# facebookresearch/visual_inertial_bundle_adjustment

Hardware: AMD Instinct MI355X
Metric: LM iterations/sec on 10k-pose/300k-landmark VI-BA (higher is better)
Workload: dtype f64; 1 GPU; config C: 5941186 obs, 300000 landmarks, 10000 rigs, reduced order 150483; rigs=10000, landmarks=300000, observations=5941186, parallelism=single GPU

## Files before the change

### visual_inertial_bundle_adjustment_amd/csrc/api.hip

```cpp
#include "host.hpp"

namespace viba {
ProfSlot g_prof;
}

namespace viba_host {

enum { KF_VISUAL_LIN = 0, KF_LANDMARK, KF_SCHUR, KF_POTRF, KF_GEMM, KF_FWD, KF_BWD, KF_BACKSUB, KF_VISUAL_COST,
       KF_SMALL, KF_TRSM, KF_SYMV, KF_COUNT };

inline void profBegin(vb_handle h, int fam) {
  if (h->profFamily != fam) return;
  if (h->profUsed + 2 > h->profEv.size()) {
    for (int i = 0; i < 256; i++) {
      hipEvent_t e;
      (void)hipEventCreate(&e);
      h->profEv.push_back(e);
    }
  }
  g_prof.start = h->profEv[h->profUsed], g_prof.stop = h->profEv[h->profUsed + 1], g_prof.consumed = false;
}
inline void profEnd(vb_handle h, int fam) {
  if (h->profFamily != fam) return;
  if (g_prof.consumed) h->profUsed += 2;
// ... 370 lines not shown
                          h->st));
    Dev g = d;
    g.tiles = h->tilesGS;
    const Sched& S = h->sch[0];
    launch_potrf(g, S.potrfTileD, S.potrfColD, (int)S.lvP[S.nLevels], h->dinv, h->st);
    launch_trsm(g, S.trsmDiagD, S.trsmTargetD, S.trsmColD, (int)S.lvT[S.nLevels], h->dinv, h->st);
    launch_diag_inverse(g, S.potrfColD, S.lvP[S.nLevels], h->linv, h->st);
  } else if (h->solverType == VB_SOLVER_PCG_LOWER_PREC) {
    return lpInit(h);
  }
  return 0;
}

int precondApply(vb_handle h, const double* r, double* z) {
  Dev& d = h->d;
  const size_t bytes = (size_t)d.nT * TS * sizeof(double);
  if (h->solverType == VB_SOLVER_PCG_GAUSS_SEIDEL) {
    HIPCHK(hipMemcpyAsync(h->pcgB, r, bytes, hipMemcpyDeviceToDevice, h->st));
    Dev g = d;
    g.tiles = h->tilesGS;
    const Sched& S = h->sch[0];
    launch_solve_fanout(g, S.tasksFD, S.nF, S.tasksBD, S.nB, S.expFD, S.expBD, h->colTilesD, h->colRowsD, h->rowTilesD,
                        h->rowColD, h->linv, h->pcgB, h->yvec, z, h->solveFlags, h->numCUs, h->st, 3,
                        nullptr, 0);
    return 0;
  }
  if (h->solverType == VB_SOLVER_PCG_LOWER_PREC) {
    lpApply(h, r, z);
    return 0;
  }
  HIPCHK(hipMemcpyAsync(z, r, bytes, hipMemcpyDeviceToDevice, h->st));
  if (h->solverType == VB_SOLVER_PCG_JACOBI) launch_jacobi_apply(d, h->jacL, r, z, h->st);
  return 0;
}

int pcgSolve(vb_handle h) {
  Dev& d = h->d;
  const int64_t n = (int64_t)d.nT * TS;
  const size_t bytes = (size_t)n * sizeof(double);
  double* x = d.xRed;
  double *r = h->pcgR, *z = h->pcgZ, *p = h->pcgP, *Ap = h->pcgAp;
  const int batch = h->solverType == VB_SOLVER_PCG_GAUSS_SEIDEL ? 1 : 8;
  HIPCHK(hipMemsetAsync(x, 0, bytes, h->st));
  HIPCHK(hipMemsetAsync(Ap, 0, bytes, h->st));
  HIPCHK(hipMemcpyAsync(r, h->rhsWork, bytes, hipMemcpyDeviceToDevice, h->st));
  if (int rc = precondApply(h, r, z)) return rc;
  HIPCHK(hipMemcpyAsync(p, z, bytes, hipMemcpyDeviceToDevice, h->st));
  HIPCHK(hipMemsetAsync(d.red + 32, 0, 12 * sizeof(double), h->st));
  launch_dot(r, r, n, d.red + 33, h->st);
  launch_dot(z, r, n, d.red + 36, h->st);
  double r02 = 0;
  if (int rc = readRed(h, &r02, 33, 1)) return rc;
  const double r0 = std::sqrt(r02);
  HIPCHK(hipMemsetAsync(d.red + 33, 0, sizeof(double), h->st));
  for (int k = 0;; k++) {
    const int zr = 36 + (k & 1), zrNew = 36 + ((k + 1) & 1);
    profBegin(h, KF_SYMV);
    launch_tile_symv(d.tiles, h->symvTilesD, h->symvRCD, h->nSymv, p, Ap, d.red + 40, h->st);
    profEnd(h, KF_SYMV);
    launch_dot(p, Ap, n, d.red + 32, h->st);
    launch_pcg_xr(x, r, p, Ap, d.red, zr, 32, n, d.red + 33, h->st);
    launch_pcg_check(d.red, r0, h->pcgTol, k, h->pcgMaxIt, zrNew, h->st);
    if (int rc = precondApply(h, r, z)) return rc;
    launch_dot(z, r, n, d.red + zrNew, h->st);
    launch_pcg_p(p, Ap, z, d.red, zrNew, zr, n, h->st);
    if ((k + 1) % batch == 0 || k + 1 >= h->pcgMaxIt) {
      double stop[3];
      if (int rc = readRed(h, stop, 40, 3)) return rc;
      if (stop[0] != 0.0) {
        h->pcgIters = (int32_t)stop[1], h->pcgRelRes = stop[2];
        return checkErr(h);
      }
      if (k + 1 >= h->pcgMaxIt) return fail(VB_E_HIP, "PCG: no stop after pcgMaxIterations");
    }
  }
}

double elapsed(hipEvent_t a, hipEvent_t b) { return profPairMs(a, b); }

}

extern "C" {

const char* vb_last_error(void) { return g_err.c_str(); }
int vb_factor_num_vars(int k) { return (k >= 0 && k < 14) ? kNumVars[k] : -1; }
int vb_factor_num_consts(int k) { return (k >= 0 && k < 14) ? kNumConsts[k] : -1; }

void vb_default_config(vb_config* c) {
  c->reproj_loss_radius = 1.0, c->reproj_loss_cutoff = 3.0;
  c->imu_loss_radius = INFINITY, c->imu_loss_cutoff = INFINITY;
  c->imu_calib_options = VB_IMU_OPT_ALL, c->device = 0, c->tile = 0, c->reserved = 0;
}
void vb_default_settings(vb_settings* s) {
  s->max_num_iterations = 50, s->stop_if_no_improvement_for = 3, s->distance_from_troubled_iteration = 3;
  s->max_step_factor_attempts = 2, s->try_sub_step = 1, s->verbose = 0;
  s->absolute_cost_tolerance = 1e-8, s->relative_cost_tolerance = 1e-10, s->variables_tolerance = 1e-5;
  s->damping = 1e-5, s->damping_adjust_on_fail = 2.5, s->damping_adjust_on_good_step = 0.7;
  s->damping_adjust_on_average_step = 1.5, s->damping_max = 1e8, s->damping_min = 1e-9;
  s->min_relative_cost_reduction = 0.3, s->step_factor_decrease = 0.3, s->min_step_factor_for_good = 0.7;
}

int vb_create(const vb_config* cfg, vb_handle* out) {
  if (!out) return fail(VB_E_ARG, "null output handle");
  int ndev = 0;
  if (hipGetDeviceCount(&ndev) != hipSuccess || ndev == 0) return fail(VB_E_HIP, "no HIP device available");
  vb_config c;
  if (cfg) c = *cfg;
  else vb_default_config(&c);
  if (c.tile != 0 && c.tile != TS) return fail(VB_E_UNSUPPORTED, "only tile size 64 is built");
  if (c.device < 0 || c.device >= ndev) return fail(VB_E_ARG, "bad device ordinal");
  HIPCHK(hipSetDevice(c.device));
  vb_handle h = new vb_handle_s();
  h->cfg = c;
  if (const char* e = getenv("VIBA_SPEC_EARLY")) h->specEarly = e[0] != '0';
  if (const char* e = getenv("VIBA_COST_FUSE")) h->costFuse = e[0] != '0';
  if (const char* e = getenv("VIBA_CLEAR_IN_FACTOR")) h->clearInFactor = e[0] != '0';
  if (const char* e = getenv("VIBA_DEBUG_SPEC_FAIL")) h->specFailDebug = e[0] == '1';
  if (const char* e = getenv("VIBA_SUPERNODE")) h->useSn = e[0] == '1';
  if (const char* e = getenv("VIBA_SN_STREAMS")) h->snStreams = std::max(1, std::min(4, atoi(e)));
  {
    hipDeviceProp_t prop;
    if (hipGetDeviceProperties(&prop, c.device) == hipSuccess && prop.multiProcessorCount > 0)
      h->numCUs = prop.multiProcessorCount;
  }
  HIPCHK(hipStreamCreateWithFlags(&h->st, hipStreamNonBlocking));
  HIPCHK(hipStreamCreateWithFlags(&h->st2, hipStreamNonBlocking));
  for (auto& e : h->ev) HIPCHK(hipEventCreate(&e));
  HIPCHK(hipEventCreateWithFlags(&h->evFork, hipEventDisableTiming));
  HIPCHK(hipEventCreateWithFlags(&h->evJoin, hipEventDisableTiming));
  HIPCHK(hipStreamCreateWithFlags(&h->stZ, hipStreamNonBlocking));
  HIPCHK(hipEventCreateWithFlags(&h->evZero, hipEventDisableTiming));
  HIPCHK(hipEventCreateWithFlags(&h->evSmallE, hipEventDisableTiming));
  HIPCHK(hipEventCreateWithFlags(&h->evZJoin, hipEventDisableTiming));
  HIPCHK(hipStreamCreateWithFlags(&h->stF, hipStreamNonBlocking));
  HIPCHK(hipEventCreateWithFlags(&h->evSnFork, hipEventDisableTiming));
  HIPCHK(hipEventCreateWithFlags(&h->evClr, hipEventDisableTiming));
  HIPCHK(hipEventCreateWithFlags(&h->evClrDone, hipEventDisableTiming));
  HIPCHK(hipEventCreateWithFlags(&h->evInvDone, hipEventDisableTiming));
  for (auto& e : h->evInvAt) HIPCHK(hipEventCreateWithFlags(&e, hipEventDisableTiming));
  HIPCHK(hipEventCreateWithFlags(&h->evStep, hipEventDisableTiming));
  HIPCHK(hipEventCreateWithFlags(&h->evRs, hipEventDisableTiming));
  for (auto& e : h->evSnLvl) HIPCHK(hipEventCreateWithFlags(&e, hipEventDisableTiming));
  *out = h;
  return 0;
}

int vb_destroy(vb_handle h) {
  if (!h) return 0;
  hipSetDevice(h->cfg.device);
  hipStreamSynchronize(h->st);
  reportFree(h);
  Dev& d = h->d;
  void* ptrs[] = {d.rvKind, d.rvHandle, d.rvDim, d.rvOff, d.rvRowEnd, d.obCostOrder, d.obPack, d.obCP, d.obPose, d.obExtr, d.obIntr, d.obVel,
                  d.obRS, d.obPt, d.obRed, d.obCol, d.obC, d.cache, d.Jt, d.lmObs, d.lmY, d.lmBlk, d.blkRed,
                  d.blkCol, d.pcRow, d.pcBlk, d.bxStart, d.bxEnt, d.Vchol, d.gp, d.z, d.xp, d.Y, d.yZero, d.gpNew, d.zNew, d.ptLm, d.oxStart, d.oxObs, d.oxSlot,
                  d.lxStart, d.lxLm, d.lxCol, d.lxChunk, d.tileWorks, d.schurRuns, d.schurTasks, d.tileEnts, d.grpStart, d.grpObs, d.grpRed, d.tileIdx, d.tiles, d.gRed, d.rhs, d.xRed, d.gRedNew, d.stepRed,
                  d.stepPt, d.subRed, d.subPt, d.lmList, d.rsOff, d.rsS, d.rsI, d.rsG, d.rsN, d.imuT, d.imuV, d.rsMid, d.rsHalf,
                  d.rsCalib, d.red, d.redS, d.err, h->colTilesD,
                  h->colRowsD, h->rowTilesD, h->rowColD, h->padRowsD, h->colStartD, h->rowStartD, h->solveFlags, h->rootTilesD, h->rootRowsD, h->rootPack, h->rowPack, h->ownRowsD, h->ownPack, h->shardTilesD, h->shardPack, (void*)h->d.colOwner, h->dinv, h->yvec,
                  h->rhsWork, h->linv, h->lscr, h->lscrSn, h->refStartD, h->refObsD, h->refPtD, h->refBackD, h->refAccD,
                  h->symvTilesD, h->symvRCD, h->pcgR, h->pcgZ, h->pcgP, h->pcgAp, h->pcgB, h->jacL, h->tilesGS, h->lpTiles, h->lpLinv, h->lpT, h->clearTilesD,
                  (void*)h->pi.src, (void*)h->pi.t, (void*)h->pi.v, (void*)h->pi.off, (void*)h->pi.noise,
                  h->tilesAlt, h->cacheAlt, h->gRedAlt, h->rsSAlt, h->rsIAlt, h->rsGAlt, h->rsNAlt};
  for (void* p : ptrs)
    if (p) hipFree(p);
  for (int k = 0; k < 9; k++) {
    if (d.var[k]) hipFree(d.var[k]);
    if (d.varBak[k]) hipFree(d.varBak[k]);
    if (d.redOf[k]) hipFree(d.redOf[k]);
  }
  for (int k = 0; k < 14; k++) {
    if (d.sf[k].vars) hipFree(d.sf[k].vars);
    if (d.sf[k].consts) hipFree(d.sf[k].consts);
  }
  {
    if (d.sJ) hipFree(d.sJ);
    if (d.sE) hipFree(d.sE);
    if (d.sMeta) hipFree(d.sMeta);
  }
  for (auto& e : h->ev) hipEventDestroy(e);
  if (h->evFork) hipEventDestroy(h->evFork);
  if (h->evJoin) hipEventDestroy(h->evJoin);
  if (h->st2) hipStreamSynchronize(h->st2), hipStreamDestroy(h->st2);
  if (h->evZero) hipEventDestroy(h->evZero);
  if (h->evSmallE) hipEventDestroy(h->evSmallE);
  if (h->evZJoin) hipEventDestroy(h->evZJoin);
  if (h->stZ) hipStreamSynchronize(h->stZ), hipStreamDestroy(h->stZ);
  if (h->stF) hipStreamSynchronize(h->stF), hipStreamDestroy(h->stF);
  if (h->evSnFork) hipEventDestroy(h->evSnFork);
  if (h->evClr) hipEventDestroy(h->evClr);
  if (h->evClrDone) hipEventDestroy(h->evClrDone);
  if (h->evInvDone) hipEventDestroy(h->evInvDone);
  for (auto& e : h->evInvAt)
    if (e) hipEventDestroy(e);
  if (h->evStep) hipEventDestroy(h->evStep);
  if (h->evRs) hipEventDestroy(h->evRs);
  for (hipEvent_t e : h->evSnLvl)
    if (e) hipEventDestroy(e);
  for (auto& e : h->profEv) hipEventDestroy(e);
  if (h->evCost) hipEventDestroy(h->evCost);
  for (auto& row : h->evS)
    for (hipEvent_t e : row)
      if (e) hipEventDestroy(e);
  if (h->stR) hipStreamSynchronize(h->stR), hipStreamDestroy(h->stR);
  if (h->hostRed) hipHostFree(h->hostRed);
  for (SnSched& N : h->sn) {
    for (void* p : {(void*)N.updD, (void*)N.fanPairsD, (void*)N.potD, (void*)N.rowD, (void*)N.fusD, (void*)N.copyD,
                    (void*)N.invEarlyD, (void*)N.invLateD})
      if (p) hipFree(p);
    for (hipGraphExec_t g : N.graph)
      if (g) hipGraphExecDestroy(g);
  }
  for (Sched& S : h->sch) {
    void* sp[] = {S.ptfD, S.ptfDiagD, S.potrfTileD, S.potrfColD, S.trsmDiagD, S.trsmTargetD, S.trsmColD, S.trsmRowD, S.updD, S.fanPairsD,
                  S.tasksFD, S.tasksBD, S.expFD, S.expBD, S.preReadyD};
    for (void* p : sp)
      if (p) hipFree(p);
    for (hipGraphExec_t g : S.graph)
      if (g) hipGraphExecDestroy(g);
  }
  hipStreamDestroy(h->st);
  delete h;
  return 0;
}

int vb_set_vars(vb_handle h, int kind, int64_t n, const double* data, const uint8_t* constant) {
  if (!h || kind < 0 || kind >= 9 || n < 0 || (n > 0 && !data)) return fail(VB_E_ARG, "bad vb_set_vars arguments");
  if (h->finalized) return fail(VB_E_STATE, "vb_set_vars after vb_finalize");
  h->data[kind].assign(data, data + n * kVarData[kind]);
  h->cst[kind].assign(n, 0);
  if (constant) std::copy(constant, constant + n, h->cst[kind].begin());
  return 0;
}

int vb_add_factors(vb_handle h, int kind, int64_t n, const int32_t* var_idx, const int32_t* ivals,
                   const double* consts) {
  if (!h || kind < 0 || kind >= 14 || n < 0 || (n > 0 && (!var_idx || !consts)))
    return fail(VB_E_ARG, "bad vb_add_factors arguments");
  if (h->finalized) return fail(VB_E_STATE, "vb_add_factors after vb_finalize");
  h->fvars[kind].insert(h->fvars[kind].end(), var_idx, var_idx + n * kNumVars[kind]);
  for (int64_t i = 0; i < n; i++) h->fint[kind].push_back(ivals ? ivals[i] : -1);
  h->fconst[kind].insert(h->fconst[kind].end(), consts, consts + n * kNumConsts[kind]);
  return 0;
}

int vb_set_rs_tables(vb_handle h, int32_t nt, const int64_t* offsets, const double* samples, const double* interp,
                     const double* gravity) {
  if (!h || nt < 0) return fail(VB_E_ARG, "bad vb_set_rs_tables arguments");
  if (h->finalized) return fail(VB_E_STATE, "vb_set_rs_tables after vb_finalize");
  if (h->rsDevice) return fail(VB_E_STATE, "vb_set_rs_tables after vb_set_rs_rigs (tables are rebuilt on the device)");
  h->nRS = nt;
  h->rsOff.assign(offsets, offsets + nt + 1);
  const int64_t ns = offsets[nt];
  h->rsS.assign(samples, samples + ns * 11);
  h->rsI.assign(interp, interp + (ns - nt) * 9);
  h->rsG.assign(gravity, gravity + nt * 3);
  for (int t = 0; t < nt; t++)
    if (offsets[t + 1] - offsets[t] < 2) return fail(VB_E_ARG, "RS table needs >= 2 samples");
  return 0;
}

int vb_set_imu_measurements(vb_handle h, int64_t n, const int64_t* timestamp_ns, const double* gyro,
                             const double* accel) {
  if (!h || n < 0 || (n && (!timestamp_ns || !gyro || !accel))) return fail(VB_E_ARG, "bad vb_set_imu_measurements arguments");
  if (h->finalized) return fail(VB_E_STATE, "vb_set_imu_measurements after vb_finalize");
  h->imuT.assign(timestamp_ns, timestamp_ns + n);
  h->imuV.resize((size_t)n * 6);
  for (int64_t i = 0; i < n; i++) {
    if (i && timestamp_ns[i] <= timestamp_ns[i - 1]) return fail(VB_E_ARG, "IMU timestamps must increase");
    for (int k = 0; k < 3; k++) h->imuV[6 * i + k] = gyro[3 * i + k], h->imuV[6 * i + 3 + k] = accel[3 * i + k];
  }
  return 0;
}

int vb_set_rs_rigs(vb_handle h, int32_t nt, const int64_t* mid_us, const int64_t* half_us, const int32_t* imu_calib,
                   int32_t gravity_var) {
  if (!h || nt < 0 || (nt && (!mid_us || !half_us || !imu_calib))) return fail(VB_E_ARG, "bad vb_set_rs_rigs arguments");
  if (h->finalized) return fail(VB_E_STATE, "vb_set_rs_rigs after vb_finalize");
  if (h->imuT.empty() && nt) return fail(VB_E_STATE, "vb_set_rs_rigs needs vb_set_imu_measurements first");
  const int64_t nCalib = (int64_t)h->data[6].size() / 32, nGrav = (int64_t)h->data[8].size() / 4;
  if (gravity_var < 0 || gravity_var >= nGrav) return fail(VB_E_ARG, "vb_set_rs_rigs: unknown gravity variable");
  for (int32_t t = 0; t < nt; t++) {
    if (imu_calib[t] < 0 || imu_calib[t] >= nCalib) return fail(VB_E_ARG, "vb_set_rs_rigs: unknown IMU calibration");
    if (half_us[t] <= 0) return fail(VB_E_ARG, "vb_set_rs_rigs: half length must be positive");
  }
  h->nRS = nt;
  h->rsMid.assign(mid_us, mid_us + nt);
  h->rsHalf.assign(half_us, half_us + nt);
  h->rsCalib.assign(imu_calib, imu_calib + nt);
  h->rsGravVar = gravity_var;
  h->rsDevice = true;
  h->rsS.clear(), h->rsI.clear(), h->rsG.clear(), h->rsOff.clear();
  return 0;
}

int rsUpdateAsync(vb_handle h, bool tables, bool preint) {
  HIPCHK(hipMemsetAsync(h->d.err + 1, 0, sizeof(int32_t), h->st));
  HIPCHK(hipEventRecord(h->ev[8], h->st));
  if (tables) launch_rs_build(h->d, h->st);
  if (preint) launch_preint(h->d, h->pi, h->st);
  HIPCHK(hipEventRecord(h->ev[9], h->st));
  h->rsTimed = true;
  return 0;
}

int vb_update_rs_tables(vb_handle h) {
  if (!h || !h->finalized) return fail(VB_E_STATE, "vb_update_rs_tables before vb_finalize");
// ... 894 lines not shown
```

### visual_inertial_bundle_adjustment_amd/csrc/device_math.hpp

```cpp
#pragma once
#include <hip/hip_runtime.h>

namespace viba {
namespace dev {

#define DEVI __device__ __forceinline__

struct q4 {
  double x, y, z, w;
};
struct v3 {
  double x, y, z;
};
struct m3 {
  double a[3][3];
};

DEVI v3 mk(double x, double y, double z) { return v3{x, y, z}; }
DEVI v3 add(v3 a, v3 b) { return {a.x + b.x, a.y + b.y, a.z + b.z}; }
DEVI v3 sub(v3 a, v3 b) { return {a.x - b.x, a.y - b.y, a.z - b.z}; }
DEVI v3 scl(double s, v3 a) { return {s * a.x, s * a.y, s * a.z}; }
DEVI v3 neg(v3 a) { return {-a.x, -a.y, -a.z}; }
DEVI double dot(v3 a, v3 b) { return a.x * b.x + a.y * b.y + a.z * b.z; }
DEVI v3 cross(v3 a, v3 b) { return {a.y * b.z - a.z * b.y, a.z * b.x - a.x * b.z, a.x * b.y - a.y * b.x}; }

DEVI q4 qmul(q4 a, q4 b) {
  q4 r;
  r.w = a.w * b.w - a.x * b.x - a.y * b.y - a.z * b.z;
  r.x = a.w * b.x + a.x * b.w + a.y * b.z - a.z * b.y;
  r.y = a.w * b.y + a.y * b.w + a.z * b.x - a.x * b.z;
  r.z = a.w * b.z + a.z * b.w + a.x * b.y - a.y * b.x;
  const double sq = r.x * r.x + r.y * r.y + r.z * r.z + r.w * r.w;
  if (sq != 1.0) {
    const double s = 2.0 / (1.0 + sq);
    r.x *= s, r.y *= s, r.z *= s, r.w *= s;
  }
  return r;
}
DEVI q4 qinv(q4 a) { return {-a.x, -a.y, -a.z, a.w}; }
DEVI v3 qrot(q4 q, v3 p) {
  v3 u{q.x, q.y, q.z};
  v3 t = scl(2.0, cross(u, p));
  return add(add(p, scl(q.w, t)), cross(u, t));
}
DEVI m3 qmat(q4 q) {
  m3 R;
  const double tx = 2 * q.x, ty = 2 * q.y, tz = 2 * q.z;
  const double twx = tx * q.w, twy = ty * q.w, twz = tz * q.w;
  const double txx = tx * q.x, txy = ty * q.x, txz = tz * q.x;
  const double tyy = ty * q.y, tyz = tz * q.y, tzz = tz * q.z;
  R.a[0][0] = 1 - (tyy + tzz), R.a[0][1] = txy - twz, R.a[0][2] = txz + twy;
  R.a[1][0] = txy + twz, R.a[1][1] = 1 - (txx + tzz), R.a[1][2] = tyz - twx;
  R.a[2][0] = txz - twy, R.a[2][1] = tyz + twx, R.a[2][2] = 1 - (txx + tyy);
  return R;
}
DEVI q4 qexp(v3 w) {
  const double th2 = dot(w, w);
  double im, re;
  if (th2 < 1e-20) {
    const double th4 = th2 * th2;
    im = 0.5 - (1.0 / 48.0) * th2 + (1.0 / 3840.0) * th4;
    re = 1.0 - (1.0 / 8.0) * th2 + (1.0 / 384.0) * th4;
  } else {
    const double th = sqrt(th2);
    double s, c;
    sincos(0.5 * th, &s, &c);
    im = s / th;
    re = c;
  }
  return {im * w.x, im * w.y, im * w.z, re};
}
DEVI v3 qlog(q4 q) {
  const double sqn = q.x * q.x + q.y * q.y + q.z * q.z;
  double f;
  if (sqn < 1e-20) {
    f = 2.0 / q.w - (2.0 / 3.0) * sqn / (q.w * q.w * q.w);
  } else {
    const double n = sqrt(sqn);
    if (fabs(q.w) < 1e-10) f = (q.w > 0 ? M_PI : -M_PI) / n;
    else f = 2.0 * atan(n / q.w) / n;
  }
  return {f * q.x, f * q.y, f * q.z};
}

DEVI m3 mmul(const m3& A, const m3& B) {
  m3 C;
#pragma unroll
  for (int i = 0; i < 3; i++)
#pragma unroll
    for (int j = 0; j < 3; j++) C.a[i][j] = A.a[i][0] * B.a[0][j] + A.a[i][1] * B.a[1][j] + A.a[i][2] * B.a[2][j];
  return C;
}
DEVI m3 hat(v3 w) {
  m3 H;
  H.a[0][0] = 0, H.a[0][1] = -w.z, H.a[0][2] = w.y;
  H.a[1][0] = w.z, H.a[1][1] = 0, H.a[1][2] = -w.x;
  H.a[2][0] = -w.y, H.a[2][1] = w.x, H.a[2][2] = 0;
  return H;
}
DEVI v3 mv(const m3& M, v3 v) {
  return {M.a[0][0] * v.x + M.a[0][1] * v.y + M.a[0][2] * v.z, M.a[1][0] * v.x + M.a[1][1] * v.y + M.a[1][2] * v.z,
          M.a[2][0] * v.x + M.a[2][1] * v.y + M.a[2][2] * v.z};
}
DEVI m3 mT(const m3& M) {
  m3 T;
#pragma unroll
  for (int i = 0; i < 3; i++)
#pragma unroll
    for (int j = 0; j < 3; j++) T.a[i][j] = M.a[j][i];
  return T;
}
DEVI m3 eye3() {
  m3 I = {};
  I.a[0][0] = I.a[1][1] = I.a[2][2] = 1.0;
  return I;
}
DEVI m3 madd(const m3& A, const m3& B, double s = 1.0) {
  m3 C;
#pragma unroll
  for (int i = 0; i < 3; i++)
#pragma unroll
    for (int j = 0; j < 3; j++) C.a[i][j] = A.a[i][j] + s * B.a[i][j];
  return C;
}

DEVI m3 so3_leftJac(v3 w) {
  const double th2 = dot(w, w);
  m3 O = hat(w), O2 = mmul(O, O);
  if (th2 < 1e-10) return madd(eye3(), O, 0.5);
  const double th = sqrt(th2);
  return madd(madd(eye3(), O, (1.0 - cos(th)) / th2), O2, (th - sin(th)) / (th2 * th));
}
DEVI m3 so3_leftJacInv(v3 w) {
  const double th2 = dot(w, w);
  m3 O = hat(w), O2 = mmul(O, O);
  m3 J = madd(eye3(), O, -0.5);
  if (th2 < 1e-10) return madd(J, O2, 1.0 / 12.0);
  const double th = sqrt(th2), h = 0.5 * th;
  return madd(J, O2, (1.0 - 0.5 * th * cos(h) / sin(h)) / th2);
}

struct se3 {
  q4 R;
  v3 t;
};
DEVI se3 se3_load(const double* d) { return {{d[0], d[1], d[2], d[3]}, {d[4], d[5], d[6]}}; }
DEVI void se3_store(const se3& T, double* d) {
  d[0] = T.R.x, d[1] = T.R.y, d[2] = T.R.z, d[3] = T.R.w, d[4] = T.t.x, d[5] = T.t.y, d[6] = T.t.z;
}
DEVI se3 se3_mul(const se3& A, const se3& B) { return {qmul(A.R, B.R), add(A.t, qrot(A.R, B.t))}; }
DEVI se3 se3_inv(const se3& A) {
  q4 ri = qinv(A.R);
  return {ri, neg(qrot(ri, A.t))};
}
DEVI v3 se3_act(const se3& A, v3 p) { return add(qrot(A.R, p), A.t); }
DEVI se3 se3_exp(const double* a) {
  v3 u{a[0], a[1], a[2]}, w{a[3], a[4], a[5]};
  return {qexp(w), mv(so3_leftJac(w), u)};
}
DEVI void se3_log(const se3& T, double* out) {
  v3 w = qlog(T.R);
  v3 u = mv(so3_leftJacInv(w), T.t);
  out[0] = u.x, out[1] = u.y, out[2] = u.z, out[3] = w.x, out[4] = w.y, out[5] = w.z;
}

DEVI m3 se3_Q(v3 ups, v3 om) {
  const double th2 = dot(om, om);
  double c1, c2, c3;
  if (th2 < 1e-4) {
    c1 = 1.0 / 6.0 - th2 / 120.0 + th2 * th2 / 5040.0;
    c2 = 1.0 / 24.0 - th2 / 720.0 + th2 * th2 / 40320.0;
    c3 = 1.0 / 120.0 - th2 / 2520.0 + th2 * th2 / 120960.0;
  } else {
    const double th = sqrt(th2), s = sin(th), c = cos(th);
    c1 = (th - s) / (th2 * th);
    c2 = (th2 + 2.0 * c - 2.0) / (2.0 * th2 * th2);
    c3 = (2.0 * th - 3.0 * s + th * c) / (2.0 * th2 * th2 * th);
  }
  m3 U = hat(ups), O = hat(om);
  m3 OU = mmul(O, U), UO = mmul(U, O), OUO = mmul(OU, O), O2 = mmul(O, O);
  m3 Q;
#pragma unroll
  for (int i = 0; i < 3; i++)
#pragma unroll
    for (int j = 0; j < 3; j++) Q.a[i][j] = 0.5 * U.a[i][j];
  m3 t1 = madd(madd(OU, UO), OUO);
  m3 t2 = madd(madd(mmul(O2, U), mmul(U, O2)), OUO, -3.0);
  m3 t3 = madd(mmul(OUO, O), mmul(O2, UO));
  Q = madd(madd(madd(Q, t1, c1), t2, c2), t3, c3);
  return Q;
}
DEVI void se3_leftJacInv(const double* a, double* M) {
  v3 u{a[0], a[1], a[2]}, w{a[3], a[4], a[5]};
  m3 Ji = so3_leftJacInv(w);
  m3 Q = se3_Q(u, w);
  m3 B = mmul(mmul(Ji, Q), Ji);
#pragma unroll
  for (int i = 0; i < 6; i++)
#pragma unroll
    for (int j = 0; j < 6; j++) M[i * 6 + j] = 0.0;
#pragma unroll
  for (int i = 0; i < 3; i++)
#pragma unroll
    for (int j = 0; j < 3; j++) {
      M[i * 6 + j] = Ji.a[i][j];
      M[(i + 3) * 6 + j + 3] = Ji.a[i][j];
      M[i * 6 + j + 3] = -B.a[i][j];
    }
}
DEVI void se3_Adj(const se3& T, double* A) {
  m3 R = qmat(T.R);
  m3 tR = mmul(hat(T.t), R);
#pragma unroll
  for (int i = 0; i < 3; i++)
#pragma unroll
    for (int j = 0; j < 3; j++) {
      A[i * 6 + j] = R.a[i][j];
      A[(i + 3) * 6 + j + 3] = R.a[i][j];
      A[i * 6 + j + 3] = tR.a[i][j];
      A[(i + 3) * 6 + j] = 0.0;
    }
}

template <bool WantJ>
DEVI bool project(const double* cam, v3 pc, double uv[2], double Jc[6], double Jp[30]) {
  if (pc.z < 1e-6) return false;
  const double iz = 1.0 / pc.z;
  const double x = pc.x * iz, y = pc.y * iz;
  const double d00 = iz, d02 = -pc.x * iz * iz, d11 = iz, d12 = -pc.y * iz * iz;
  const double* p = cam + 9;
  if (cam[0] == 0.0) {
    uv[0] = p[0] * x + p[2];
    uv[1] = p[1] * y + p[3];
    if (WantJ) {
      Jc[0] = p[0] * d00, Jc[1] = 0.0, Jc[2] = p[0] * d02;
      Jc[3] = 0.0, Jc[4] = p[1] * d11, Jc[5] = p[1] * d12;
#pragma unroll
      for (int i = 0; i < 30; i++) Jp[i] = 0.0;
      Jp[0] = x, Jp[2] = 1;
      Jp[16] = y, Jp[18] = 1;
    }
    return true;
  }
  const double f = p[0];
  const double p0 = p[9], p1 = p[10];
  const double r2 = x * x + y * y, r = sqrt(r2);
  const double th = atan(r), th2 = th * th;
  double R = 1.0, dR = 0.0, t2i = th2;
  double thp[6];
#pragma unroll
  for (int i = 0; i < 6; i++) {
    thp[i] = t2i;
    R += p[3 + i] * t2i;
    dR += p[3 + i] * 2.0 * (i + 1) * t2i;
    t2i *= th2;
  }
  double g, gpr;
  if (r < 1e-8) {
    g = 1.0;
    gpr = 2.0 * (p[3] - 1.0 / 3.0);
  } else {
    dR /= th;
    const double thr = th / r, dth = 1.0 / (1.0 + r2);
    g = R * thr;
    gpr = ((dR * dth * th + R * dth) / r - R * th / r2) / r;
  }
  const double xr = g * x, yr = g * y;
  const double rr2 = xr * xr + yr * yr, rr4 = rr2 * rr2;
  const double tmp = 2.0 * (xr * p0 + yr * p1);
  const double ud = xr + tmp * xr + rr2 * p0 + p[11] * rr2 + p[12] * rr4;
  const double vd = yr + tmp * yr + rr2 * p1 + p[13] * rr2 + p[14] * rr4;
  uv[0] = f * ud + p[1];
  uv[1] = f * vd + p[2];
  if (WantJ) {
    const double a0 = p[11] + 2.0 * p[12] * rr2, a1 = p[13] + 2.0 * p[14] * rr2;
    const double D00 = 1.0 + 6.0 * xr * p0 + 2.0 * yr * p1 + 2.0 * xr * a0;
    const double D01 = 2.0 * p1 * xr + 2.0 * yr * p0 + 2.0 * yr * a0;
    const double D10 = 2.0 * p0 * yr + 2.0 * xr * p1 + 2.0 * xr * a1;
    const double D11 = 1.0 + 2.0 * xr * p0 + 6.0 * yr * p1 + 2.0 * yr * a1;
    const double G00 = g + x * x * gpr, G01 = x * y * gpr, G11 = g + y * y * gpr;
    const double M00 = f * (D00 * G00 + D01 * G01), M01 = f * (D00 * G01 + D01 * G11);
    const double M10 = f * (D10 * G00 + D11 * G01), M11 = f * (D10 * G01 + D11 * G11);
    Jc[0] = M00 * d00, Jc[1] = M01 * d11, Jc[2] = M00 * d02 + M01 * d12;
    Jc[3] = M10 * d00, Jc[4] = M11 * d11, Jc[5] = M10 * d02 + M11 * d12;
    Jp[0] = ud, Jp[15] = vd;
    Jp[1] = 1, Jp[16] = 0, Jp[2] = 0, Jp[17] = 1;
    const double thdivr = (r < 1e-8) ? 1.0 : th / r;
#pragma unroll
    for (int i = 0; i < 6; i++) {
      const double dxr = thdivr * thp[i] * x, dyr = thdivr * thp[i] * y;
      Jp[3 + i] = f * (D00 * dxr + D01 * dyr);
      Jp[18 + i] = f * (D10 * dxr + D11 * dyr);
    }
    Jp[9] = f * (2.0 * xr * xr + rr2), Jp[24] = f * (2.0 * xr * yr);
    Jp[10] = f * (2.0 * xr * yr), Jp[25] = f * (2.0 * yr * yr + rr2);
    Jp[11] = f * rr2, Jp[12] = f * rr4, Jp[13] = 0, Jp[14] = 0;
    Jp[26] = 0, Jp[27] = 0, Jp[28] = f * rr2, Jp[29] = f * rr4;
  }
  return true;
}

struct rvp {
  q4 R;
  v3 dV, dP;
  double dt;
};
DEVI rvp integrate(v3 gyro, v3 accel, double dt) {
  v3 om = scl(dt, gyro), ups = scl(dt, accel);
  rvp o;
  o.R = qexp(om);
  const double th2 = dot(om, om), th = sqrt(th2), th4 = th2 * th2;
  double c1, c2, c3;
  if (th < 1e-3) {
    c1 = (1.0 / 2.0) - (th2 / 24.0) + (th4 / 729.0);
    c2 = (1.0 / 6.0) - (th2 / 120.0) + (th4 / 5040.0);
    c3 = (1.0 / 24.0) - (th2 / 729.0) + (th4 / 40320.0);
  } else {
    const double sT = sin(th) / th, mC = (1.0 - cos(th)) / th2;
    c1 = mC, c2 = (1.0 - sT) / th2, c3 = (0.5 - mC) / th2;
  }
  m3 O = hat(om), O2 = mmul(O, O);
  m3 U2V = madd(madd(eye3(), O, c1), O2, c2);
  o.dV = mv(U2V, ups);
  m3 U2P = madd(madd(madd(eye3(), eye3(), -0.5), O, c2), O2, c3);
  o.dP = mv(U2P, scl(dt, ups));
  o.dt = dt;
  return o;
}
DEVI rvp combine(const rvp& a, const rvp& b) {
  rvp c;
  c.R = qmul(a.R, b.R);
  c.dV = add(a.dV, qrot(a.R, b.dV));
  c.dP = add(add(a.dP, scl(b.dt, a.dV)), qrot(a.R, b.dP));
  c.dt = a.dt + b.dt;
  return c;
}

DEVI rvp uncombine_left(const rvp& c, const rvp& a) {
  const q4 ai = qinv(a.R);
  rvp b;
  b.R = qmul(ai, c.R);
  b.dV = qrot(ai, sub(c.dV, a.dV));
  b.dt = c.dt - a.dt;
  b.dP = qrot(ai, sub(sub(c.dP, a.dP), scl(b.dt, a.dV)));
  return b;
}
DEVI v3 vdiv(v3 a, double s) { return {a.x / s, a.y / s, a.z / s}; }
DEVI void differentiate(const rvp& r, double* out) {
  const v3 om = qlog(r.R);
  const double th2 = dot(om, om), th = sqrt(th2);
  double q2;
  if (th < 1e-3) {
    q2 = 1.0 / 12.0 - th2 / (4.0 * 180.0) + (th2 * th2) / (16.0 * 1890.0);
  } else {
    const double h = th * 0.5;
    q2 = (1.0 - h * cos(h) / sin(h)) / th2;
  }
  const v3 ov = cross(om, r.dV);
  const v3 ups = add(add(r.dV, scl(-0.5, ov)), scl(q2, cross(om, ov)));
  const v3 g = vdiv(om, r.dt), a = vdiv(ups, r.dt);
  const rvp rec = integrate(g, a, r.dt);
  const v3 dv = vdiv(sub(r.dP, rec.dP), r.dt);
  out[0] = g.x, out[1] = g.y, out[2] = g.z, out[3] = a.x, out[4] = a.y, out[5] = a.z;
  out[6] = dv.x, out[7] = dv.y, out[8] = dv.z;
}

DEVI se3 rs_estimate(const double* samples, const double* interp, int n, const double* grav,
                     double tDelta, v3 velW, q4 R_b_w, bool* outOfRange) {
  int lo = 0, hi = n;
  while (lo < hi) {
    const int mid = (lo + hi) >> 1;
    if (tDelta < samples[mid * 11 + 10]) hi = mid;
    else lo = mid + 1;
  }
  const int idx = lo;
  if (idx == n || idx == 0) {
    *outOfRange = true;
    return {{0, 0, 0, 1}, {0, 0, 0}};
  }
  const double* s = samples + (idx - 1) * 11;
  const double* ip = interp + (idx - 1) * 9;
  rvp prev{{s[0], s[1], s[2], s[3]}, {s[4], s[5], s[6]}, {s[7], s[8], s[9]}, s[10]};
  const double dtl = tDelta - prev.dt;
  rvp inc = integrate(mk(ip[0], ip[1], ip[2]), mk(ip[3], ip[4], ip[5]), dtl);
  inc.dP = add(inc.dP, scl(dtl, mk(ip[6], ip[7], ip[8])));
  rvp atT = combine(prev, inc);
  v3 gMid = qrot(R_b_w, mk(grav[0], grav[1], grav[2]));
  v3 vMid = qrot(R_b_w, velW);
  v3 pos = add(add(atT.dP, scl(tDelta, vMid)), scl(0.5 * tDelta * tDelta, gMid));
  return {atT.R, pos};
}

DEVI void huber_jet2(double a, double b, double k2, double h, double s, double& v, double& d) {
  if (!(s > b)) {
    v = s, d = 1.0;
  } else if (s > k2) {
    v = h, d = 0.0;
  } else {
    const double r = sqrt(s);
    d = a / r;
    v = 2.0 * a * r - b;
  }
}
DEVI double huber_val(double a, double b, double k2, double h, double s) {
  if (!(s > b)) return s;
  if (s > k2) return h;
  return 2.0 * a * sqrt(s) - b;
}

}
}
```

### visual_inertial_bundle_adjustment_amd/csrc/engine.hpp

```cpp
#pragma once
#include <hip/hip_ext.h>
#include <hip/hip_runtime.h>
#include <cstdint>
#include <cstddef>
#include <cstdlib>

namespace viba {

#ifndef VIBA_MIXED
#define VIBA_MIXED 0
#endif
#if VIBA_MIXED
typedef float rec_t;
#else
typedef double rec_t;
#endif

constexpr int kLmSmallCols = 256;

constexpr int kJe = 0;
constexpr int kJpt = 2;
constexpr int kJpose = 8;
constexpr int kJextr = 20;
constexpr int kJintr = 32;
constexpr int kJvel = 66;
constexpr int kJPlanes = 72;
constexpr int kJA = 32, kJB = 40;
template <typename T>
__host__ __device__ inline T* jt_plane(T* Jt, int64_t nPad, int64_t o, int plane) {
  return plane < kJA ? Jt + o * kJA + plane : Jt + nPad * kJA + o * kJB + (plane - kJA);
}
constexpr int kSlotPose = 0, kSlotExtr = 1, kSlotIntr = 2, kSlotVel = 3;
__host__ __device__ inline int slotPlane(int s) {
  return s == 0 ? kJpose : s == 1 ? kJextr : s == 2 ? kJintr : kJvel;
}
__host__ __device__ inline int slotStride(int s) { return s == 0 || s == 1 ? 6 : s == 2 ? 17 : 3; }

struct ImuIdx {
  int gB, aB, gS, aS, gN, aN, rT, gaT, size;
};

struct PreintSrc {
  int32_t kind, imu;
  int64_t row, t0Us, t1Us;
};
struct PreintArgs {
  const PreintSrc* src = nullptr;
  int64_t n = 0;
  const int64_t* t = nullptr;
  const double* v = nullptr;
  const int64_t* off = nullptr;
  const double* noise = nullptr;
};

struct LossParams {
  double a, b, k2, h;
};

struct SmallFactors {
  int64_t n = 0;
  int32_t* vars = nullptr;
  double* consts = nullptr;
  int nv = 0, nc = 0;
  int64_t stage = 0;
};
constexpr int kSmallRows = 23, kSmallCols = 80;
constexpr int kSmallJ = kSmallRows * kSmallCols, kSmallE = 24, kSmallMeta = 36;

struct TileEnt {
  uint32_t colI, colJ;
  uint16_t nI, nJ;
  uint32_t lm;
  uint64_t maskI, maskJ;
};
struct TileWork {
  int32_t tile, I, J, count;
  int64_t start;
  int32_t kind, pad;
  int32_t runFirst, taskFirst;
  uint16_t nRuns, wOff[5];
};
#ifndef VIBA_SCHUR_TR
#define VIBA_SCHUR_TR (VIBA_MIXED ? 2 : 1)
#endif
constexpr int kSchurCh = 24, kSchurTR = VIBA_SCHUR_TR;

struct Dev {
  double* var[9] = {};
  double* varBak[9] = {};
  int64_t nvar[9] = {};
  int32_t* redOf[9] = {};
  int32_t nRV = 0;
  int64_t nRed = 0;
  int32_t* rvKind = nullptr;
  int32_t* rvHandle = nullptr;
  int32_t* rvDim = nullptr;
  int64_t* rvOff = nullptr;
  int64_t* rvRowEnd = nullptr;
  int64_t nObs = 0, nObsPad = 0;
  int32_t *obPose = nullptr, *obExtr = nullptr, *obIntr = nullptr, *obVel = nullptr,
          *obRS = nullptr, *obPt = nullptr;
  int32_t* obRed = nullptr;
  int32_t* obCostOrder = nullptr;
  int32_t* obPack = nullptr;
  double* obCP = nullptr;
  int32_t* obCol = nullptr;
  double* obC = nullptr;
  double* cache = nullptr;
  double* cacheW = nullptr;
  rec_t* Jt = nullptr;
  int64_t nPts = 0;
  int64_t* lmObs = nullptr;
  int64_t* lmY = nullptr;
  int64_t* lmBlk = nullptr;
  int32_t* blkRed = nullptr;
  int32_t* blkCol = nullptr;
  int32_t* pcRow = nullptr;
  int64_t nYcol = 0;
  int32_t* pcBlk = nullptr;
  int64_t* bxStart = nullptr;
  int32_t* bxEnt = nullptr;
  double *Vchol = nullptr, *gp = nullptr, *z = nullptr, *xp = nullptr;
  rec_t* yZero = nullptr;
  rec_t* Y = nullptr;
  double *gpNew = nullptr, *zNew = nullptr;
  int32_t* ptRed = nullptr;
  int32_t* ptLm = nullptr;
  int64_t* oxStart = nullptr;
  int32_t* oxObs = nullptr;
  int32_t* oxSlot = nullptr;
  int64_t* lxStart = nullptr;
  int32_t* lxLm = nullptr;
  int32_t* lxCol = nullptr;
  int64_t* lxChunk = nullptr;
  int64_t nLxChunk = 0;
  int64_t nTileWorks = 0;
  TileWork* tileWorks = nullptr;
  uint64_t* schurRuns = nullptr;
  uint32_t* schurTasks = nullptr;
  TileEnt* tileEnts = nullptr;
  int64_t nGroups = 0;
  int64_t* grpStart = nullptr;
  int32_t* grpObs = nullptr;
  int32_t* grpRed = nullptr;
  int T = 64;
  int32_t nT = 0;
  int64_t nTiles = 0;
  int32_t* tileIdx = nullptr;
  double* tiles = nullptr;
  int64_t* colStart = nullptr;
  double *gRed = nullptr, *rhs = nullptr, *xRed = nullptr, *gRedNew = nullptr;
  double *stepRed = nullptr, *stepPt = nullptr, *subRed = nullptr, *subPt = nullptr;
  SmallFactors sf[14];
  int64_t nSmallStage = 0;
  double* sJ = nullptr;
  double* sE = nullptr;
  int32_t* sMeta = nullptr;
  int32_t nRS = 0;
  int64_t* rsOff = nullptr;
  int32_t* rsN = nullptr;
  double *rsS = nullptr, *rsI = nullptr, *rsG = nullptr;
  int64_t nImu = 0;
  int64_t* imuT = nullptr;
  double* imuV = nullptr;
  int64_t *rsMid = nullptr, *rsHalf = nullptr;
  int32_t* rsCalib = nullptr;
  int32_t rsGravVar = 0;
  double* red = nullptr;
  double* redS = nullptr;
  double* costS = nullptr;
  int32_t* err = nullptr;
  int64_t lmB = 0, lmE = 0, obB = 0, obE = 0, obFree = 0, fB = 0, fE = 0;
  int32_t* lmList = nullptr;
  int64_t nLmSmall = 0, nLmBig = 0;
  int32_t lmBigCols = 0;
  int32_t root = 1;
  const int8_t* colOwner = nullptr;
  int32_t myRank = 0, world = 1;
  LossParams reproj, imu;
  ImuIdx jac;
};

__device__ __forceinline__ bool owns_col(const Dev& d, int64_t col) {
  if (d.world <= 1) return true;
  const int o = d.colOwner[col];
  return o == d.myRank || (o == d.world && d.myRank == 0);
}

struct ProfSlot {
  hipEvent_t start = nullptr, stop = nullptr;
  bool consumed = false;
};
extern ProfSlot g_prof;

template <typename K, typename... Args>
inline void launchK(K kernel, dim3 grid, dim3 block, uint32_t shmem, hipStream_t st, Args... args) {
  if (g_prof.start && !g_prof.consumed) {
    hipExtLaunchKernelGGL(kernel, grid, block, shmem, st, g_prof.start, g_prof.stop, 0, args...);
    g_prof.consumed = true;
  } else {
    hipLaunchKernelGGL(kernel, grid, block, shmem, st, args...);
  }
}

}
```

### visual_inertial_bundle_adjustment_amd/csrc/factors.hip

```cpp
#include "device_math.hpp"
#include "engine.hpp"
#include "report.hpp"
#include <algorithm>

namespace viba {
using namespace dev;

__device__ __forceinline__ v3 mk3(const double* base, int h) {
  const double* p = base + (int64_t)h * 3;
  return mk(p[0], p[1], p[2]);
}

template <int N>
__device__ void block_sum_atomic(double (&v)[N], double* out) {
  __shared__ double sh[N][4];
#pragma unroll
  for (int k = 0; k < N; k++) {
    double x = v[k];
#pragma unroll
    for (int off = 32; off > 0; off >>= 1) x += __shfl_down(x, off, 64);
    if ((threadIdx.x & 63) == 0) sh[k][threadIdx.x >> 6] = x;
  }
  __syncthreads();
  if (threadIdx.x == 0) {
    const int nw = (blockDim.x + 63) >> 6;
#pragma unroll
    for (int k = 0; k < N; k++) {
      double s = 0;
      for (int w = 0; w < nw; w++) s += sh[k][w];
      if (s != 0.0) atomicAdd(out + k, s);
    }
  }
}

struct VisOut {
  double e[2];
  double Jpt[6], Jpose[12], Jextr[12], Jvel[6];
  double* Jintr;
};

template <bool WantJ, bool PointOnly = false>
__device__ bool vis_eval(const double* obsC, v3 X, const se3& Tbw, const se3& Tcb, const double* cam,
                         VisOut& o) {
  v3 pRig = se3_act(Tbw, X);
  v3 pCam = se3_act(Tcb, pRig);
  double uv[2], Jc[6], Jp[30];
  if (!project<WantJ>(cam, pCam, uv, Jc, Jp)) return false;
  const double s00 = obsC[2], s01 = obsC[3], s10 = obsC[4], s11 = obsC[5];
  const double r0 = uv[0] - obsC[0], r1 = uv[1] - obsC[1];
  o.e[0] = s00 * r0 + s01 * r1;
  o.e[1] = s10 * r0 + s11 * r1;
  if (WantJ) {
    double dW[6];
#pragma unroll
    for (int j = 0; j < 3; j++) dW[j] = s00 * Jc[j] + s01 * Jc[3 + j], dW[3 + j] = s10 * Jc[j] + s11 * Jc[3 + j];
    m3 Rcb = qmat(Tcb.R);
    m3 Rcw = qmat(qmul(Tcb.R, Tbw.R));
#pragma unroll
    for (int r = 0; r < 2; r++) {
#pragma unroll
      for (int j = 0; j < 3; j++)
        o.Jpt[r * 3 + j] = dW[r * 3] * Rcw.a[0][j] + dW[r * 3 + 1] * Rcw.a[1][j] + dW[r * 3 + 2] * Rcw.a[2][j];
      if (PointOnly) continue;
      double A[3];
#pragma unroll
      for (int j = 0; j < 3; j++)
        A[j] = dW[r * 3] * Rcb.a[0][j] + dW[r * 3 + 1] * Rcb.a[1][j] + dW[r * 3 + 2] * Rcb.a[2][j];
      const v3 mp = neg(pRig);
      o.Jpose[r * 6 + 0] = A[0], o.Jpose[r * 6 + 1] = A[1], o.Jpose[r * 6 + 2] = A[2];
      o.Jpose[r * 6 + 3] = A[1] * mp.z - A[2] * mp.y;
      o.Jpose[r * 6 + 4] = -A[0] * mp.z + A[2] * mp.x;
      o.Jpose[r * 6 + 5] = A[0] * mp.y - A[1] * mp.x;
      const v3 mc = neg(pCam);
      const double* B = dW + r * 3;
      o.Jextr[r * 6 + 0] = B[0], o.Jextr[r * 6 + 1] = B[1], o.Jextr[r * 6 + 2] = B[2];
      o.Jextr[r * 6 + 3] = B[1] * mc.z - B[2] * mc.y;
      o.Jextr[r * 6 + 4] = -B[0] * mc.z + B[2] * mc.x;
      o.Jextr[r * 6 + 5] = B[0] * mc.y - B[1] * mc.x;
    }
    if (PointOnly) return true;
    const int n = (int)cam[1];
#pragma unroll
    for (int j = 0; j < 17; j++) {
      const bool in = j < 15 && j < n;
      const double a0 = in ? Jp[j < 15 ? j : 0] : 0.0, a1 = in ? Jp[15 + (j < 15 ? j : 0)] : 0.0;
      o.Jintr[j] = s00 * a0 + s01 * a1;
      o.Jintr[17 + j] = s10 * a0 + s11 * a1;
    }
  }
  return true;
}

template <bool WantJ, bool PointOnly = false>
__device__ bool rs_eval(const Dev& d, const double* obsC, int rs, v3 X, const se3& Tbw, const se3& Tcb,
                        const double* cam, v3 vel, bool wantTime, bool wantVel, VisOut& o, bool* oor) {
  const double tpf = obsC[1] / cam[3] - 0.5;
  const double ro = cam[4] != 0.0 ? cam[5] : 0.0;
  const double dt = ro * tpf - cam[6];
  const int64_t s0 = d.rsOff[rs], ns = d.rsN[rs];
  const double* S = d.rsS + s0 * 11;
  const double* I = d.rsI + (s0 - rs) * 9;
  const double* G = d.rsG + rs * 3;
  se3 Twb = se3_inv(Tbw);
  q4 Rbw = qinv(Twb.R);
  se3 TmidAtT = rs_estimate(S, I, (int)ns, G, dt, vel, Rbw, oor);
  if (*oor) return false;
  se3 TAtTMid = se3_inv(TmidAtT);
  se3 TAtTw = se3_mul(TAtTMid, Tbw);
  if (!vis_eval<WantJ, PointOnly>(obsC, X, TAtTw, Tcb, cam, o)) return false;
  if (WantJ && !PointOnly) {
    double Jt[12];
#pragma unroll
    for (int i = 0; i < 12; i++) Jt[i] = o.Jpose[i];
    const int n = (int)cam[1];
    const bool estRO = cam[7] != 0.0, estOff = cam[8] != 0.0;
    if (wantTime && (estRO || estOff)) {
      const double kEps = 1e-6;
      se3 TP = rs_estimate(S, I, (int)ns, G, dt + kEps, vel, Rbw, oor);
      if (*oor) return false;
      se3 dd = se3_mul(se3_inv(TP), TmidAtT);
      double lg[6];
      se3_log(dd, lg);
      double dE[2];
#pragma unroll
      for (int r = 0; r < 2; r++) {
        double s = 0;
#pragma unroll
        for (int k = 0; k < 6; k++) s += Jt[r * 6 + k] * (lg[k] / kEps);
        dE[r] = s;
      }
      const int iRO = estRO ? n : -1, iOff = estOff ? n + (estRO ? 1 : 0) : -1;
#pragma unroll
      for (int j = 0; j < 17; j++) {
        if (j == iOff) o.Jintr[j] = -dE[0], o.Jintr[17 + j] = -dE[1];
        if (j == iRO) o.Jintr[j] = dE[0] * tpf, o.Jintr[17 + j] = dE[1] * tpf;
      }
    }
    double M[36];
    se3_Adj(TAtTMid, M);
    v3 vv = add(scl(dt, vel), scl(0.5 * dt * dt, mk(G[0], G[1], G[2])));
    m3 H = hat(qrot(TAtTw.R, vv));
#pragma unroll
    for (int i = 0; i < 3; i++)
#pragma unroll
      for (int j = 0; j < 3; j++) M[i * 6 + 3 + j] += H.a[i][j];
#pragma unroll
    for (int r = 0; r < 2; r++)
#pragma unroll
      for (int j = 0; j < 6; j++) {
        double s = 0;
#pragma unroll
        for (int k = 0; k < 6; k++) s += Jt[r * 6 + k] * M[k * 6 + j];
        o.Jpose[r * 6 + j] = s;
      }
    if (wantVel) {
      m3 R = qmat(TAtTw.R);
#pragma unroll
      for (int r = 0; r < 2; r++)
#pragma unroll
        for (int j = 0; j < 3; j++)
          o.Jvel[r * 3 + j] = -dt * (Jt[r * 6] * R.a[0][j] + Jt[r * 6 + 1] * R.a[1][j] + Jt[r * 6 + 2] * R.a[2][j]);
    } else {
#pragma unroll
      for (int i = 0; i < 6; i++) o.Jvel[i] = 0.0;
    }
  }
  return true;
}

typedef double double2_t __attribute__((ext_vector_type(2)));
typedef float float2_t __attribute__((ext_vector_type(2)));
__device__ __forceinline__ void store_planes(double* p, double a, double b) { *(double2_t*)p = double2_t{a, b}; }
__device__ __forceinline__ void store_planes(float* p, double a, double b) { *(float2_t*)p = float2_t{(float)a, (float)b}; }
constexpr int kVisBlock = 128;

template <bool Cost>
__global__ void __launch_bounds__(kVisBlock) visual_lin_kernel(Dev d, int updateCache, int dontRetry, int64_t lo,
                                                               int64_t hi) {
  __shared__ double stage[kVisBlock / 64][64 * kJB];
  const int lane = threadIdx.x & 63, wave = threadIdx.x >> 6;
  const int64_t ob = lo + (int64_t)blockIdx.x * kVisBlock + wave * 64;
  const int nrec = (int)max<int64_t>(0, min<int64_t>(64, hi - ob));
  int4 pa = make_int4(0, 0, 0, 0), pb = make_int4(0, 0, 0, 0);
  if (lane < nrec) pa = reinterpret_cast<const int4*>(d.obPack)[2 * (ob + lane)], pb = reinterpret_cast<const int4*>(d.obPack)[2 * (ob + lane) + 1];
  const int32_t o = pa.x;
  double* S = stage[wave];
  double acc[1] = {0.0};
  double cst[4] = {0.0, 0.0, 0.0, 0.0};
  VisOut v;
  v.Jintr = S + lane * kJB;
  bool ok = false;
  double w = 0.0;
  if (lane < nrec) {
    ok = true;
    bool oor = false;
    const double c0 = d.cache[o];
    if (dontRetry && c0 < 0.0) {
      ok = false;
      if (updateCache) d.cacheW[o] = c0;
    } else {
      const double* obsC = d.obCP + (ob + lane) * 6;
      const double* Xp = d.var[0] + (int64_t)pa.y * 3;
      v3 X = mk(Xp[0], Xp[1], Xp[2]);
      se3 Tbw = se3_load(d.var[1] + (int64_t)pa.z * 7);
      se3 Tcb = se3_load(d.var[5] + (int64_t)pa.w * 7);
      const double* cam = d.var[4] + (int64_t)pb.x * 24;
      const int rs = pb.y;
      if (rs < 0) {
        ok = vis_eval<true>(obsC, X, Tbw, Tcb, cam, v);
#pragma unroll
        for (int i = 0; i < 6; i++) v.Jvel[i] = 0.0;
      } else {
        const double* vp = d.var[2] + (int64_t)pb.z * 3;
        ok = rs_eval<true>(d, obsC, rs, X, Tbw, Tcb, cam, mk(vp[0], vp[1], vp[2]), (pb.w & 1) != 0,
                           (pb.w & 2) != 0, v, &oor);
        if (oor) atomicOr(d.err, 1);
      }
      if (!ok && (updateCache || dontRetry)) (updateCache ? d.cacheW : d.cache)[o] = -1.0;
    }
    if (ok) {
      const double s = v.e[0] * v.e[0] + v.e[1] * v.e[1];
      double rho, drho;
      huber_jet2(d.reproj.a, d.reproj.b, d.reproj.k2, d.reproj.h, s, rho, drho);
      w = sqrt(drho);
      acc[0] = 0.5 * rho;
      if (updateCache) d.cacheW[o] = 0.5 * rho;
    }
    if (Cost && pb.y < 0) {
      const bool prevInvalid = c0 < 0.0;
      cst[1] = 1.0;
      cst[2] = ok ? 0.0 : 1.0;
      cst[3] = prevInvalid ? 1.0 : 0.0;
      cst[0] = prevInvalid ? 0.0 : (ok ? acc[0] : c0);
    }
  }
  if (lane < nrec) {
    double* r = S + lane * kJB;
#pragma unroll
    for (int i = 0; i < 34; i++) r[i] = ok ? w * r[i] : 0.0;
#pragma unroll
    for (int i = 0; i < 6; i++) r[kJvel - kJA + i] = ok ? w * v.Jvel[i] : 0.0;
  }
  __builtin_amdgcn_fence(__ATOMIC_RELEASE, "wavefront");
  __builtin_amdgcn_wave_barrier();
  __builtin_amdgcn_fence(__ATOMIC_ACQUIRE, "wavefront");
  {
    rec_t* dst = d.Jt + d.nObsPad * kJA;
    const int nq = nrec * (kJB / 2);
    for (int q0 = 0; q0 < nq; q0 += 64) {
      const int q = q0 + lane, r = min(q / (kJB / 2), 63), c = 2 * (q % (kJB / 2));
      const int64_t orec = __shfl(o, r, 64);
      if (q < nq) store_planes(dst + orec * kJB + c, S[r * kJB + c], S[r * kJB + c + 1]);
    }
  }
  __builtin_amdgcn_fence(__ATOMIC_RELEASE, "wavefront");
  __builtin_amdgcn_wave_barrier();
  __builtin_amdgcn_fence(__ATOMIC_ACQUIRE, "wavefront");
  if (lane < nrec) {
    double* r = S + lane * (kJA + 1);
#pragma unroll
    for (int i = 0; i < 2; i++) r[kJe + i] = ok ? w * v.e[i] : 0.0;
#pragma unroll
    for (int i = 0; i < 6; i++) r[kJpt + i] = ok ? w * v.Jpt[i] : 0.0;
#pragma unroll
    for (int i = 0; i < 12; i++) r[kJpose + i] = ok ? w * v.Jpose[i] : 0.0;
#pragma unroll
    for (int i = 0; i < 12; i++) r[kJextr + i] = ok ? w * v.Jextr[i] : 0.0;
  }
  __builtin_amdgcn_fence(__ATOMIC_RELEASE, "wavefront");
  __builtin_amdgcn_wave_barrier();
  __builtin_amdgcn_fence(__ATOMIC_ACQUIRE, "wavefront");
  {
    const int nq = nrec * (kJA / 2);
    for (int q0 = 0; q0 < nq; q0 += 64) {
      const int q = q0 + lane, r = min(q / (kJA / 2), 63), c = 2 * (q % (kJA / 2));
      const int64_t orec = __shfl(o, r, 64);
      if (q < nq) store_planes(d.Jt + orec * kJA + c, S[r * (kJA + 1) + c], S[r * (kJA + 1) + c + 1]);
    }
  }
  double x = acc[0];
#pragma unroll
  for (int off = 32; off > 0; off >>= 1) x += __shfl_down(x, off, 64);
  if (lane == 0 && x != 0.0) atomicAdd(d.redS + (blockIdx.x & 63) * 8 + 0, x);
  if (Cost) {
#pragma unroll
    for (int k = 0; k < 4; k++) {
      double y = cst[k];
#pragma unroll
      for (int off = 32; off > 0; off >>= 1) y += __shfl_down(y, off, 64);
      if (lane == 0 && y != 0.0) atomicAdd(d.costS + (blockIdx.x & 63) * 8 + 1 + k, y);
    }
  }
}

__global__ void __launch_bounds__(256) visual_cost_kernel(Dev d, int comparable, int64_t lo, int64_t hi) {
  const int64_t i = lo + (int64_t)blockIdx.x * blockDim.x + threadIdx.x;
  double acc[4] = {0.0, 0.0, 0.0, 0.0};
  if (i < hi) {
    const int4 pa = reinterpret_cast<const int4*>(d.obPack)[2 * i], pb = reinterpret_cast<const int4*>(d.obPack)[2 * i + 1];
    const int64_t o = pa.x;
    VisOut v;
    v.Jintr = nullptr;
    bool oor = false, ok;
    const double* obsC = d.obCP + i * 6;
    const double* Xp = d.var[0] + (int64_t)pa.y * 3;
    v3 X = mk(Xp[0], Xp[1], Xp[2]);
    se3 Tbw = se3_load(d.var[1] + (int64_t)pa.z * 7);
    se3 Tcb = se3_load(d.var[5] + (int64_t)pa.w * 7);
    const double* cam = d.var[4] + (int64_t)pb.x * 24;
    const int rs = pb.y;
    if (rs < 0) {
      ok = vis_eval<false>(obsC, X, Tbw, Tcb, cam, v);
    } else {
      const double* vp = d.var[2] + (int64_t)pb.z * 3;
      ok = rs_eval<false>(d, obsC, rs, X, Tbw, Tcb, cam, mk(vp[0], vp[1], vp[2]), false, false, v, &oor);
      if (oor) atomicOr(d.err, 32);
    }
    const double prev = d.cache[o];
    const bool prevInvalid = prev < 0.0;
    acc[1] = 1.0;
    acc[2] = ok ? 0.0 : 1.0;
    acc[3] = prevInvalid ? 1.0 : 0.0;
    if (comparable && prevInvalid) {
    } else if (comparable && !ok) {
      acc[0] = prev;
    } else if (ok) {
      const double s = v.e[0] * v.e[0] + v.e[1] * v.e[1];
      acc[0] = 0.5 * huber_val(d.reproj.a, d.reproj.b, d.reproj.k2, d.reproj.h, s);
    }
  }
  block_sum_atomic<4>(acc, d.redS + (blockIdx.x & 63) * 8 + 1);
}

template <bool Hist>
__global__ void __launch_bounds__(256) visual_report_kernel(Dev d, const int32_t* posOfRow, RepRows R, RepHist H,
                                                            int32_t* err) {
  __shared__ RepTable tab;
  if (Hist) rep_clear(tab, H);
  const int64_t n = Hist ? d.nObs : R.n;
  for (int64_t t = (int64_t)blockIdx.x * 256 + threadIdx.x; t < n; t += (int64_t)gridDim.x * 256) {
    const int64_t i = Hist ? t : posOfRow[R.first + t];
    const int4 pa = reinterpret_cast<const int4*>(d.obPack)[2 * i], pb = reinterpret_cast<const int4*>(d.obPack)[2 * i + 1];
    VisOut v;
    v.Jintr = nullptr;
    v.e[0] = v.e[1] = 0.0;
    bool oor = false, ok;
    const double* obsC = d.obCP + i * 6;
    const double* Xp = d.var[0] + (int64_t)pa.y * 3;
    v3 X = mk(Xp[0], Xp[1], Xp[2]);
    se3 Tbw = se3_load(d.var[1] + (int64_t)pa.z * 7);
    se3 Tcb = se3_load(d.var[5] + (int64_t)pa.w * 7);
    const double* cam = d.var[4] + (int64_t)pb.x * 24;
    const int rs = pb.y;
    if (rs < 0) {
      ok = vis_eval<false>(obsC, X, Tbw, Tcb, cam, v);
    } else {
      const double* vp = d.var[2] + (int64_t)pb.z * 3;
      ok = rs_eval<false>(d, obsC, rs, X, Tbw, Tcb, cam, mk(vp[0], vp[1], vp[2]), false, false, v, &oor);
      if (oor) atomicOr(err, 1);
    }
    const double s = ok ? v.e[0] * v.e[0] + v.e[1] * v.e[1] : 0.0;
    const double cost = ok ? 0.5 * huber_val(d.reproj.a, d.reproj.b, d.reproj.k2, d.reproj.h, s) : 0.0;
    if (Hist) {
      rep_add(tab, H, H.grp ? H.grp[i] : 0, ok, sqrt(2.0 * (0.5 * s)), cost);
    } else {
      if (R.raw) R.raw[2 * t] = ok ? v.e[0] : 0.0, R.raw[2 * t + 1] = ok ? v.e[1] : 0.0;
      if (R.squ) R.squ[t] = 0.5 * s;
      if (R.sqw) R.sqw[t] = 0.5 * s;
      if (R.cost) R.cost[t] = cost;
      if (R.valid) R.valid[t] = ok ? 1 : 0;
    }
  }
  if (Hist) rep_flush(tab, H);
}

constexpr int kMaxM = kSmallRows;
constexpr int kMaxCols = kSmallCols;

struct SmallEval {
  int m = 0;
  int nslot = 0;
  int col[10], dim[10], red[10];
  double e[kMaxM];
  double (*J)[kMaxCols];
};

__device__ inline void imu_boxminus(const double* v, const double* r, const ImuIdx& J, double* res) {
  if (J.gB >= 0) for (int i = 0; i < 3; i++) res[J.gB + i] = v[6 + i] - r[6 + i];
  if (J.aB >= 0) for (int i = 0; i < 3; i++) res[J.aB + i] = v[9 + i] - r[9 + i];
  if (J.gS >= 0) for (int i = 0; i < 3; i++) res[J.gS + i] = 1.0 / v[i] - 1.0 / r[i];
  if (J.aS >= 0) for (int i = 0; i < 3; i++) res[J.aS + i] = 1.0 / v[3 + i] - 1.0 / r[3 + i];
  if (J.gN >= 0) {
    res[J.gN + 0] = v[12 + 3] - r[12 + 3];
    res[J.gN + 1] = v[12 + 6] - r[12 + 6];
    res[J.gN + 2] = v[12 + 1] - r[12 + 1];
    res[J.gN + 3] = v[12 + 7] - r[12 + 7];
    res[J.gN + 4] = v[12 + 2] - r[12 + 2];
    res[J.gN + 5] = v[12 + 5] - r[12 + 5];
  }
  if (J.aN >= 0) {
    res[J.aN + 0] = v[21 + 3] - r[21 + 3];
    res[J.aN + 1] = v[21 + 6] - r[21 + 6];
    res[J.aN + 2] = v[21 + 7] - r[21 + 7];
  }
  if (J.rT >= 0) res[J.rT] = v[31] - r[31];
  if (J.gaT >= 0) res[J.gaT] = (v[30] - v[31]) - (r[30] - r[31]);
}

__device__ void inertial_eval(const double* c, const double* calib, const ImuIdx& jac, const se3& Tp, v3 vp,
                              const se3& Tn, v3 vn, v3 g, SmallEval& E, const int cols[5]) {
  const int n = jac.size;
  const double dt = c[10];
  double corr[9];
#pragma unroll
  for (int i = 0; i < 9; i++) corr[i] = 0.0;
  {
    const double* r = c + 11 + 207 + 81;
    const double* Jc = c + 11;
    auto take = [&](double v) {
#pragma unroll
      for (int i = 0; i < 9; i++) corr[i] += Jc[i] * v;
      Jc += 9;
    };
    if (jac.gB >= 0)
#pragma unroll
      for (int i = 0; i < 3; i++) take(calib[6 + i] - r[6 + i]);
    if (jac.aB >= 0)
#pragma unroll
      for (int i = 0; i < 3; i++) take(calib[9 + i] - r[9 + i]);
    if (jac.gS >= 0)
#pragma unroll
      for (int i = 0; i < 3; i++) take(1.0 / calib[i] - 1.0 / r[i]);
    if (jac.aS >= 0)
#pragma unroll
      for (int i = 0; i < 3; i++) take(1.0 / calib[3 + i] - 1.0 / r[3 + i]);
    if (jac.gN >= 0) {
      constexpr int kG[6] = {3, 6, 1, 7, 2, 5};
#pragma unroll
      for (int i = 0; i < 6; i++) take(calib[12 + kG[i]] - r[12 + kG[i]]);
    }
    if (jac.aN >= 0) {
      constexpr int kA[3] = {3, 6, 7};
#pragma unroll
      for (int i = 0; i < 3; i++) take(calib[21 + kA[i]] - r[21 + kA[i]]);
    }
    if (jac.rT >= 0) take(calib[31] - r[31]);
    if (jac.gaT >= 0) take((calib[30] - calib[31]) - (r[30] - r[31]));
  }
  q4 Rc = qexp(mk(-corr[0], -corr[1], -corr[2]));
  q4 cR = qmul(Rc, qinv(q4{c[0], c[1], c[2], c[3]}));
  q4 Rerr = qmul(qmul(cR, Tp.R), qinv(Tn.R));
  v3 lre = neg(qlog(Rerr));
  v3 dVp = qrot(Tp.R, sub(sub(vn, vp), scl(dt, g)));
  v3 velErr = add(sub(mk(c[4], c[5], c[6]), dVp), mk(corr[3], corr[4], corr[5]));
  q4 Rpn = qmul(Tp.R, qinv(Tn.R));
  v3 dPp = sub(sub(Tp.t, qrot(Rpn, Tn.t)), qrot(Tp.R, add(scl(dt, vp), scl(0.5 * dt * dt, g))));
  v3 posErr = add(sub(mk(c[7], c[8], c[9]), dPp), mk(corr[6], corr[7], corr[8]));
  E.e[0] = lre.x, E.e[1] = lre.y, E.e[2] = lre.z;
  E.e[3] = velErr.x, E.e[4] = velErr.y, E.e[5] = velErr.z;
  E.e[6] = posErr.x, E.e[7] = posErr.y, E.e[8] = posErr.z;
  m3 dL = so3_leftJacInv(neg(lre));
  m3 Rp = qmat(Tp.R);
  if (cols[1] >= 0) {
    const int c0 = cols[1];
    m3 A = mmul(dL, qmat(cR));
    m3 hv = hat(dVp), hp = hat(dPp);
    for (int i = 0; i < 3; i++)
      for (int j = 0; j < 3; j++) {
        E.J[i][c0 + j] = 0.0, E.J[i][c0 + 3 + j] = -A.a[i][j];
        E.J[3 + i][c0 + j] = 0.0, E.J[3 + i][c0 + 3 + j] = hv.a[i][j];
        E.J[6 + i][c0 + j] = (i == j) ? -1.0 : 0.0, E.J[6 + i][c0 + 3 + j] = hp.a[i][j];
      }
  }
  if (cols[2] >= 0) {
    const int c0 = cols[2];
    for (int i = 0; i < 3; i++)
      for (int j = 0; j < 3; j++) {
        E.J[i][c0 + j] = 0.0;
        E.J[3 + i][c0 + j] = Rp.a[i][j];
        E.J[6 + i][c0 + j] = Rp.a[i][j] * dt;
      }
  }
  if (cols[3] >= 0) {
    const int c0 = cols[3];
    m3 A = mmul(dL, qmat(Rerr));
    m3 Rm = qmat(Rpn);
    for (int i = 0; i < 3; i++)
      for (int j = 0; j < 3; j++) {
        E.J[i][c0 + j] = 0.0, E.J[i][c0 + 3 + j] = A.a[i][j];
        E.J[3 + i][c0 + j] = 0.0, E.J[3 + i][c0 + 3 + j] = 0.0;
        E.J[6 + i][c0 + j] = Rm.a[i][j], E.J[6 + i][c0 + 3 + j] = 0.0;
      }
  }
  if (cols[4] >= 0) {
    const int c0 = cols[4];
    for (int i = 0; i < 3; i++)
      for (int j = 0; j < 3; j++) {
// ... 423 lines not shown
  const int64_t slot = s0 + (int64_t)blockIdx.x * 4 + wave;
  if (slot >= s1) return;
  const int32_t* mt = d.sMeta + slot * kSmallMeta;
  const int m = mt[0], colc = mt[1], nv = mt[2], uoff = mt[3], fk = mt[4];
  const double* Jg = d.sJ + slot * kSmallJ;
  const double* se = d.sE + slot * kSmallE;
  const double drho = se[0];
  double* J = Jl[wave];
  const double* U = uoff >= 0 ? d.sf[fk].consts + uoff : nullptr;
  for (int j = lane; j < colc; j += 64) {
    double col[MM];
#pragma unroll
    for (int i = 0; i < MM; i++) col[i] = i < m ? Jg[i * kMaxCols + j] : 0.0;
    if (U) {
#pragma unroll
      for (int i = 0; i < MM; i++) {
        if (i >= m) break;
        double s = 0;
#pragma unroll
        for (int q = 0; q < MM; q++)
          if (q < m) s += U[i * m + q] * col[q];
        J[i * kMaxCols + j] = s;
      }
    } else {
#pragma unroll
      for (int i = 0; i < MM; i++)
        if (i < m) J[i * kMaxCols + j] = col[i];
    }
  }
  const int T = d.T;
  int32_t vro = 0x7fffffff, vdim = 0, vcol = 0;
  if (lane < nv) {
    const int red = mt[5 + lane];
    if (red >= 0) vro = (int32_t)d.rvOff[red], vdim = mt[25 + lane], vcol = mt[15 + lane];
  }
  int32_t vstart = 0, nAct = 0;
  for (int s = 0; s < nv; s++) {
    const int32_t ro = __builtin_amdgcn_readlane(vro, s), dim = __builtin_amdgcn_readlane(vdim, s);
    if (ro < vro) vstart += dim;
    nAct += dim;
  }
  if (nAct <= 64) {
    const bool on = lane < nAct;
    int32_t R = 0, c = 0;
    for (int s = 0; s < nv; s++) {
      const int32_t st = __builtin_amdgcn_readlane(vstart, s), dim = __builtin_amdgcn_readlane(vdim, s);
      if (lane >= st && lane < st + dim) {
        R = __builtin_amdgcn_readlane(vro, s) + (lane - st);
        c = __builtin_amdgcn_readlane(vcol, s) + (lane - st);
      }
    }
    const int32_t t = R / T;
    uint64_t left = __ballot(on);
    int nu = 0, u = -1;
    while (left) {
      const int32_t tl = __builtin_amdgcn_readlane(t, __builtin_ctzll(left));
      const bool hit = on && t == tl;
      left &= ~__ballot(hit);
      if (nu < kAsmTiles) {
        if (hit) u = nu;
        if (lane == 0) trow[wave][nu] = tl;
        nu++;
      }
    }
    if (on) act[wave][lane][0] = c, act[wave][lane][1] = R << 5 | (u + 1);
    if (lane == 0) act[wave][kMaxCols - 1][0] = nu, act[wave][kMaxCols - 1][1] = nAct;
  } else if (lane == 0) {
    int32_t vro[10], vs[10], nvar = 0;
    for (int s = 0; s < nv; s++) {
      const int red = mt[5 + s];
      if (red < 0) continue;
      const int32_t ro = (int32_t)d.rvOff[red];
      int k = nvar++;
      for (; k > 0 && vro[k - 1] > ro; k--) vro[k] = vro[k - 1], vs[k] = vs[k - 1];
      vro[k] = ro, vs[k] = s;
    }
    int n = 0, nu = 0;
    for (int k = 0; k < nvar; k++) {
      const int s = vs[k];
      for (int i = 0; i < mt[25 + s]; i++) {
        const int32_t R = vro[k] + i, t = R / T;
        int u = 0;
        while (u < nu && trow[wave][u] != t) u++;
        if (u == nu && nu < kAsmTiles) trow[wave][nu++] = t;
        act[wave][n][0] = mt[15 + s] + i, act[wave][n][1] = R << 5 | (u < kAsmTiles ? u + 1 : 0), n++;
      }
    }
    act[wave][kMaxCols - 1][0] = nu, act[wave][kMaxCols - 1][1] = n;
  }
  __builtin_amdgcn_wave_barrier();
  __builtin_amdgcn_fence(__ATOMIC_SEQ_CST, "workgroup");
  const int A = act[wave][kMaxCols - 1][1];
  for (int a = lane; a < A; a += 64) {
    const int c = act[wave][a][0];
    double g = 0;
    for (int r = 0; r < m; r++) g += J[r * kMaxCols + c] * se[1 + r];
    const int32_t R = act[wave][a][1] >> 5;
    if (owns_col(d, R / T)) atomicAdd(gOut + R, drho * g);
  }
  if (mode != 0) return;
  const int nu = act[wave][kMaxCols - 1][0];
  for (int q = lane; q < nu * nu; q += 64) {
    const int tu = trow[wave][q / nu], tv = trow[wave][q % nu];
    tpair[wave][q] = tu >= tv ? d.tileIdx[(int64_t)tu * d.nT + tv] : -1;
  }
  __builtin_amdgcn_wave_barrier();
  __builtin_amdgcn_fence(__ATOMIC_SEQ_CST, "workgroup");
  const int P = A * (A + 1) / 2;
  for (int p = lane; p < P; p += 64) {
    const int q = P - 1 - p;
    int i = (int)((sqrtf(8.0f * q + 1.0f) - 1.0f) * 0.5f);
    while (i * (i + 1) / 2 > q) i--;
    while ((i + 1) * (i + 2) / 2 <= q) i++;
    const int b = A - 1 - i, a = A - 1 - (q - i * (i + 1) / 2);
    const int ca = act[wave][a][0], cb = act[wave][b][0];
    double hs = 0;
    for (int r = 0; r < m; r++) hs += J[r * kMaxCols + ca] * J[r * kMaxCols + cb];
    const int32_t wa = act[wave][a][1], wb = act[wave][b][1];
    const int32_t R = wa >> 5, C = wb >> 5, uR = (wa & 31) - 1, uC = (wb & 31) - 1;
    if (!owns_col(d, C / T)) continue;
    double* dst = uR >= 0 && uC >= 0 ? d.tiles + (int64_t)tpair[wave][uR * nu + uC] * T * T + (C % T) * T + (R % T)
                                     : tile_addr(d, R, C);
    atomicAdd(dst, drho * hs);
  }
}

__device__ __forceinline__ double refine_wave_sum(double x) {
#pragma unroll
  for (int off = 32; off > 0; off >>= 1) x += __shfl_xor(x, off, 64);
  return x;
}

template <bool WantJ>
__device__ bool refine_eval(const Dev& d, int64_t o, v3 X, VisOut& v) {
  const double* obsC = d.obC + o * 6;
  se3 Tbw = se3_load(d.var[1] + (int64_t)d.obPose[o] * 7);
  se3 Tcb = se3_load(d.var[5] + (int64_t)d.obExtr[o] * 7);
  const double* cam = d.var[4] + (int64_t)d.obIntr[o] * 24;
  const int rs = d.obRS[o];
  if (rs < 0) return vis_eval<WantJ, true>(obsC, X, Tbw, Tcb, cam, v);
  const double* vp = d.var[2] + (int64_t)d.obVel[o] * 3;
  bool oor = false;
  const bool ok = rs_eval<WantJ, true>(d, obsC, rs, X, Tbw, Tcb, cam, mk(vp[0], vp[1], vp[2]), false, false, v, &oor);
  if (oor) atomicOr(d.err, 1);
  return ok;
}

__device__ void refine_grad_hess(const Dev& d, const int32_t* obs, int64_t n, double* bk, v3 X, bool update,
                                 double& cost, double g[3], double H[6]) {
  const int lane = threadIdx.x & 63;
  double c = 0, g0 = 0, g1 = 0, g2 = 0, h00 = 0, h10 = 0, h20 = 0, h11 = 0, h21 = 0, h22 = 0;
  for (int64_t q = lane; q < n; q += 64) {
    VisOut v;
    v.Jintr = nullptr;
    if (!refine_eval<true>(d, obs[q], X, v)) {
      if (update) bk[q] = -1.0;
      continue;
    }
    const double s = v.e[0] * v.e[0] + v.e[1] * v.e[1];
    double rho, drho;
    huber_jet2(d.reproj.a, d.reproj.b, d.reproj.k2, d.reproj.h, s, rho, drho);
    c += 0.5 * rho;
    if (update) bk[q] = 0.5 * rho;
    const double a0 = drho * v.Jpt[0], a1 = drho * v.Jpt[1], a2 = drho * v.Jpt[2];
    const double b0 = drho * v.Jpt[3], b1 = drho * v.Jpt[4], b2 = drho * v.Jpt[5];
    g0 += v.e[0] * a0 + v.e[1] * b0, g1 += v.e[0] * a1 + v.e[1] * b1, g2 += v.e[0] * a2 + v.e[1] * b2;
    h00 += a0 * v.Jpt[0] + b0 * v.Jpt[3], h10 += a1 * v.Jpt[0] + b1 * v.Jpt[3], h20 += a2 * v.Jpt[0] + b2 * v.Jpt[3];
    h11 += a1 * v.Jpt[1] + b1 * v.Jpt[4], h21 += a2 * v.Jpt[1] + b2 * v.Jpt[4], h22 += a2 * v.Jpt[2] + b2 * v.Jpt[5];
  }
  cost = refine_wave_sum(c);
  g[0] = refine_wave_sum(g0), g[1] = refine_wave_sum(g1), g[2] = refine_wave_sum(g2);
  H[0] = refine_wave_sum(h00), H[1] = refine_wave_sum(h10), H[2] = refine_wave_sum(h20);
  H[3] = refine_wave_sum(h11), H[4] = refine_wave_sum(h21), H[5] = refine_wave_sum(h22);
}

__device__ double refine_cost(const Dev& d, const int32_t* obs, int64_t n, const double* bk, v3 X) {
  const int lane = threadIdx.x & 63;
  double c = 0;
  for (int64_t q = lane; q < n; q += 64) {
    if (bk[q] < 0) continue;
    VisOut v;
    v.Jintr = nullptr;
    if (!refine_eval<false>(d, obs[q], X, v)) {
      c += bk[q];
      continue;
    }
    const double s = v.e[0] * v.e[0] + v.e[1] * v.e[1];
    c += 0.5 * huber_val(d.reproj.a, d.reproj.b, d.reproj.k2, d.reproj.h, s);
  }
  return refine_wave_sum(c);
}

__device__ void refine_ldlt_solve(const double Hl[6], const double b[3], double x[3]) {
  double m[3][3] = {{Hl[0], Hl[1], Hl[2]}, {Hl[1], Hl[3], Hl[4]}, {Hl[2], Hl[4], Hl[5]}};
  int tr[3];
  for (int k = 0; k < 3; k++) {
    int big = k;
    for (int i = k + 1; i < 3; i++)
      if (fabs(m[i][i]) > fabs(m[big][big])) big = i;
    tr[k] = big;
    if (big != k) {
      for (int j = 0; j < 3; j++) { const double t = m[k][j]; m[k][j] = m[big][j]; m[big][j] = t; }
      for (int i = 0; i < 3; i++) { const double t = m[i][k]; m[i][k] = m[i][big]; m[i][big] = t; }
    }
    double tmp[3];
    for (int j = 0; j < k; j++) tmp[j] = m[j][j] * m[k][j];
    for (int j = 0; j < k; j++) m[k][k] -= m[k][j] * tmp[j];
    for (int i = k + 1; i < 3; i++) {
      for (int j = 0; j < k; j++) m[i][k] -= m[i][j] * tmp[j];
      if (m[k][k] != 0.0) m[i][k] /= m[k][k];
    }
  }
  for (int i = 0; i < 3; i++) x[i] = b[i];
  for (int k = 0; k < 3; k++)
    if (tr[k] != k) { const double t = x[k]; x[k] = x[tr[k]]; x[tr[k]] = t; }
  for (int i = 0; i < 3; i++)
    for (int j = 0; j < i; j++) x[i] -= m[i][j] * x[j];
  for (int i = 0; i < 3; i++) x[i] = fabs(m[i][i]) > 2.2250738585072014e-308 ? x[i] / m[i][i] : 0.0;
  for (int i = 2; i >= 0; i--)
    for (int j = i + 1; j < 3; j++) x[i] -= m[j][i] * x[j];
  for (int k = 2; k >= 0; k--)
    if (tr[k] != k) { const double t = x[k]; x[k] = x[tr[k]]; x[tr[k]] = t; }
}

__global__ void __launch_bounds__(256) refine_points_kernel(Dev d, const int64_t* gStart, const int32_t* gObs,
                                                            const int32_t* gPt, int64_t nG, double* backups,
                                                            double* acc) {
  const int64_t g = (int64_t)blockIdx.x * 4 + (threadIdx.x >> 6);
  if (g >= nG) return;
  const int lane = threadIdx.x & 63;
  const int64_t q0 = gStart[g], n = gStart[g + 1] - q0;
  const int32_t* obs = gObs + q0;
  double* bk = backups + q0;
  double* Xp = d.var[0] + (int64_t)gPt[g] * 3;
  v3 X = mk(Xp[0], Xp[1], Xp[2]);
  constexpr double kLambda = 1e-5, kCostTol = 1e-8, kStepTol = 1e-6, kMinImpr = 0.2, kStepRed = 0.3;
  double startCost = 0, endCost = 0;
  int nIts = 0;
  for (int i = 0; i < 5; i++) {
    double cost, gr[3], H[6];
    refine_grad_hess(d, obs, n, bk, X, true, cost, gr, H);
    if (i == 0) startCost = endCost = cost;
    H[0] = H[0] * (1.0 + kLambda) + kLambda, H[3] = H[3] * (1.0 + kLambda) + kLambda;
    H[5] = H[5] * (1.0 + kLambda) + kLambda;
    double st[3];
    refine_ldlt_solve(H, gr, st);
    st[0] = -st[0], st[1] = -st[1], st[2] = -st[2];
    const v3 Xb = X;
    bool success = false;
    X = mk(X.x + st[0], X.y + st[1], X.z + st[2]);
    double newCost = refine_cost(d, obs, n, bk, X);
    const double modelDelta = st[0] * gr[0] + st[1] * gr[1] + st[2] * gr[2];
    if (-modelDelta < kCostTol) break;
    if (newCost < cost + modelDelta * kMinImpr) {
      success = true;
    } else {
      double nc, ng[3], nH[6];
      refine_grad_hess(d, obs, n, bk, X, false, nc, ng, nH);
      X = Xb;
      const double newDelta = st[0] * ng[0] + st[1] * ng[1] + st[2] * ng[2];
      const double f = newDelta > 0 ? -modelDelta / (newDelta - modelDelta) : kStepRed;
      st[0] *= f, st[1] *= f, st[2] *= f;
      X = mk(X.x + st[0], X.y + st[1], X.z + st[2]);
      newCost = refine_cost(d, obs, n, bk, X);
      if (newCost < cost + (st[0] * gr[0] + st[1] * gr[1] + st[2] * gr[2]) * kMinImpr) success = true;
      else X = Xb;
    }
    if (success) {
      nIts++;
      endCost = newCost;
    } else {
      nIts = -1;
      break;
    }
    if (st[0] * st[0] + st[1] * st[1] + st[2] * st[2] < kStepTol * kStepTol) break;
  }
  if (lane == 0) {
    Xp[0] = X.x, Xp[1] = X.y, Xp[2] = X.z;
    atomicAdd(acc + 0, startCost);
    atomicAdd(acc + 1, endCost);
    atomicAdd(acc + (nIts < 0 ? 2 : 3), nIts < 0 ? 1.0 : (double)nIts);
    if (nIts > 0) atomicAdd(acc + 4, 1.0);
  }
}

void launch_refine_points(const Dev& d, const int64_t* gStart, const int32_t* gObs, const int32_t* gPt, int64_t nG,
                          double* backups, double* acc, hipStream_t st) {
  if (nG > 0)
    hipLaunchKernelGGL(refine_points_kernel, dim3((unsigned)((nG + 3) / 4)), dim3(256), 0, st, d, gStart, gObs, gPt, nG,
                       backups, acc);
}

void launch_visual_lin(const Dev& d, int updateCache, int dontRetry, int64_t lo, int64_t hi, hipStream_t st) {
  if (hi <= lo) return;
  const int64_t n = hi - lo;
  if (d.costS)
    launchK(visual_lin_kernel<true>, dim3((unsigned)((n + kVisBlock - 1) / kVisBlock)), dim3(kVisBlock), 0, st, d,
            updateCache, dontRetry, lo, hi);
  else
    launchK(visual_lin_kernel<false>, dim3((unsigned)((n + kVisBlock - 1) / kVisBlock)), dim3(kVisBlock), 0, st, d,
            updateCache, dontRetry, lo, hi);
}
__global__ void fold_red_kernel(Dev d) {
  const int k = threadIdx.x;
  if (k >= 8) return;
  double s = 0.0;
  for (int i = 0; i < 64; i++) s += d.redS[i * 8 + k], d.redS[i * 8 + k] = 0.0;
  if (s != 0.0) atomicAdd(d.red + k, s);
}
void launch_fold_red(const Dev& d, hipStream_t st) { hipLaunchKernelGGL(fold_red_kernel, dim3(1), dim3(64), 0, st, d); }
struct VarCopy {
  const double* src[9];
  double* dst[9];
  int64_t off[10];
};
__global__ void __launch_bounds__(256) copy_vars_kernel(VarCopy c) {
  for (int64_t i = (int64_t)blockIdx.x * 256 + threadIdx.x; i < c.off[9]; i += (int64_t)gridDim.x * 256) {
    int k = 0;
    while (i >= c.off[k + 1]) k++;
    c.dst[k][i - c.off[k]] = c.src[k][i - c.off[k]];
  }
}
void launch_copy_vars(const Dev& d, bool backup, const int64_t* len, hipStream_t st) {
  VarCopy c{};
  c.off[0] = 0;
  for (int k = 0; k < 9; k++) {
    c.src[k] = backup ? d.var[k] : d.varBak[k];
    c.dst[k] = backup ? d.varBak[k] : d.var[k];
    c.off[k + 1] = c.off[k] + len[k];
  }
  if (c.off[9] > 0)
    hipLaunchKernelGGL(copy_vars_kernel, dim3((unsigned)std::min<int64_t>(1024, (c.off[9] + 255) / 256)), dim3(256), 0, st, c);
}
__global__ void spec_commit_kernel(Dev d) {
  const int k = threadIdx.x;
// ... 66 lines not shown
```

### visual_inertial_bundle_adjustment_amd/csrc/finalize.hip

```cpp
#include "host.hpp"

namespace viba_host {
namespace {

Knobs readKnobs(const vb_handle_s& h) {
  Knobs k;
  if (const char* e = getenv("VIBA_ND_CUTWIN")) k.cutWin = std::max(0.0, std::min(0.45, atof(e)));
  if (const char* e = getenv("VIBA_ND_LEAF")) k.leafDims = std::max<int64_t>(64, atoll(e));
  k.stats = getenv("VIBA_STATS") != nullptr;
  k.ptFuseMax = h.ptFuseMax, k.useSn = h.useSn, k.snStreams = h.snStreams;
  return k;
}

int uploadSched(const SchedHost& H, Sched& S) {
  static_cast<SchedShape&>(S) = H;
  if (upload(&S.potrfTileD, H.potrfTile) || upload(&S.potrfColD, H.potrfCol) || upload(&S.trsmDiagD, H.trsmDiag) ||
      upload(&S.trsmTargetD, H.trsmTarget) || upload(&S.trsmColD, H.trsmCol) || upload(&S.trsmRowD, H.trsmRow) ||
      upload(&S.updD, H.upd) || upload(&S.fanPairsD, H.fanPairs) || upload(&S.tasksFD, H.tasksF) ||
      upload(&S.tasksBD, H.tasksB) || upload(&S.expFD, H.expF) || upload(&S.expBD, H.expB) ||
      upload(&S.preReadyD, H.preReady) || upload(&S.ptfD, H.ptf) || upload(&S.ptfDiagD, H.ptfDiag))
    return VB_E_HIP;
  return 0;
}

int uploadSnSched(const SnSchedHost& H, SnSched& S) {
  static_cast<SnSchedShape&>(S) = H;
  if (upload(&S.updD, H.upd) || upload(&S.fanPairsD, H.fanPairs) || upload(&S.potD, H.pot) || upload(&S.rowD, H.row) ||
      upload(&S.fusD, H.fus) || upload(&S.copyD, H.copy) || upload(&S.invEarlyD, H.invEarly) ||
      upload(&S.invLateD, H.invLate))
    return VB_E_HIP;
  return 0;
}

void copyToHandle(vb_handle h, const Symbolic& A) {
  Dev& d = h->d;
  d.jac = makeJac(h->cfg.imu_calib_options);
  d.reproj = makeLoss(h->cfg.reproj_loss_radius, h->cfg.reproj_loss_cutoff);
  d.imu = makeLoss(h->cfg.imu_loss_radius, h->cfg.imu_loss_cutoff);
  d.T = TS;
  for (int k = 0; k < 9; k++) d.nvar[k] = A.reg.nvar[k];
  const int64_t nPts = A.reg.nPts;
  d.nRV = A.lay.nRV, d.nRed = A.lay.nRed, d.nPts = nPts, d.nT = A.lay.nT, d.nTiles = A.pat.nTiles;
  d.nObs = A.obs.nObs, d.nObsPad = A.obs.nObsPad, d.nYcol = A.pan.nYcol;
  d.nLxChunk = (int64_t)A.pan.lxChunk.size() / 3;
  d.lmB = A.shard.lmBegin, d.lmE = A.shard.lmEnd, d.root = A.shard.isRoot ? 1 : 0;
  d.nLmSmall = A.shard.nLmSmall, d.nLmBig = A.shard.nLmBig, d.lmBigCols = A.shard.lmBigCols;
  d.obB = A.shard.obB, d.obE = A.shard.obE, d.obFree = A.shard.obFree, d.fB = A.shard.fB, d.fE = A.shard.fE;
  d.nGroups = (int64_t)A.schur.grpRed.size() / 4;
  d.nTileWorks = (int64_t)A.schur.works.size();
  for (int fk = 1; fk < 14; fk++) {
    SmallFactors& sf = d.sf[fk];
    sf.nv = kNumVars[fk], sf.n = (int64_t)h->fint[fk].size(), sf.nc = A.small.nc[fk], sf.stage = A.small.stage[fk];
  }
  d.nSmallStage = A.small.nSmallStage;
  d.myRank = h->partRank, d.world = h->partWorld;
  d.nRS = h->nRS;

  h->rvKind = A.lay.rvKind, h->rvHandle = A.lay.rvHandle, h->rvDim = A.lay.rvDim, h->rvOff = A.lay.rvOff;
  h->lmOfPoint = A.reg.lmOfPoint;
  h->colOwner = A.lay.colOwner;
  h->nRedReal = A.lay.nRedReal, h->nParts = (int64_t)A.nd.partBegin.size();
  h->nParams = nPts + A.lay.nRV;
  h->order = nPts * 3 + A.lay.nRedReal;
  h->nPadRows = (int64_t)A.lay.padRows.size();
  h->nLmObs = A.obs.lmObs[nPts];
  h->lmBegin = A.shard.lmBegin, h->lmEnd = A.shard.lmEnd, h->isRoot = A.shard.isRoot;
  h->tileFill = A.pat.tileFill;
  h->colStart = A.pat.colStart, h->colTilesH = A.pat.colTiles, h->colRowsH = A.pat.colRows;
  h->rowStart = A.pat.rowStart, h->rowTilesH = A.pat.rowTiles, h->rowColH = A.pat.rowCol;
  h->nClear = (int64_t)A.schur.clearTiles.size();
  h->nTileEnt = (int64_t)A.schur.ents.size(), h->nObEnt = d.nGroups;
  h->tileFirst = A.schur.tileFirst, h->tileCount = A.schur.tileCount;
  h->shardTiles = A.schur.shardTiles;
  h->zeroRuns = A.part.zeroRuns, h->rootTiles = A.part.rootTiles, h->rootRows = A.part.rootRows;
  h->nOwnRows = (int64_t)A.part.ownRows.size();
  h->nLevels = A.pat.nLevels;
  h->nPairs = A.sch[0].nPairs + A.sch[1].nPairs;
  h->costRsB[0] = A.cost.rsBegin[0], h->costRsB[1] = A.cost.rsBegin[1];
  h->visRowOfPos.resize(A.cost.order.size());
  for (size_t i = 0; i < A.cost.order.size(); i++) h->visRowOfPos[i] = (int32_t)A.obs.perm[A.cost.order[i]];
  if (A.preint.present) h->piNoise = A.preint.noise;
}

int uploadRsTables(vb_handle h) {
  Dev& d = h->d;
  if (h->rsDevice) {
    const int64_t kWidenNs = 20000000;
    h->rsOff.assign(h->nRS + 1, 0);
    for (int32_t t = 0; t < h->nRS; t++) {
      const int64_t a = (h->rsMid[t] - h->rsHalf[t]) * 1000 - kWidenNs, b = (h->rsMid[t] + h->rsHalf[t]) * 1000 + kWidenNs;
      const int64_t cnt = std::upper_bound(h->imuT.begin(), h->imuT.end(), b) -
                          std::lower_bound(h->imuT.begin(), h->imuT.end(), a);
      h->rsOff[t + 1] = h->rsOff[t] + cnt + 4;
    }
    const int64_t ns = h->rsOff[h->nRS];
    std::vector<int32_t> zeroN(h->nRS, 0);
    if (upload(&d.rsOff, h->rsOff) || alloc0(&d.rsS, ns * 11) || alloc0(&d.rsI, (ns - h->nRS) * 9) ||
        alloc0(&d.rsG, (size_t)h->nRS * 3) || upload(&d.rsN, zeroN) || upload(&d.imuT, h->imuT) ||
        upload(&d.imuV, h->imuV) || upload(&d.rsMid, h->rsMid) || upload(&d.rsHalf, h->rsHalf) ||
        upload(&d.rsCalib, h->rsCalib))
      return VB_E_HIP;
    d.nImu = (int64_t)h->imuT.size();
    d.rsGravVar = h->rsGravVar;
    return 0;
  }
  std::vector<int32_t> cnt(h->nRS);
  for (int32_t t = 0; t < h->nRS; t++) cnt[t] = (int32_t)(h->rsOff[t + 1] - h->rsOff[t]);
  if (h->rsOff.empty()) h->rsOff.assign(1, 0);
  if (upload(&d.rsOff, h->rsOff) || upload(&d.rsS, h->rsS) || upload(&d.rsI, h->rsI) || upload(&d.rsG, h->rsG) ||
      upload(&d.rsN, cnt))
    return VB_E_HIP;
  return 0;
}

int uploadAll(vb_handle h, const Symbolic& A) {
  Dev& d = h->d;
  const int64_t nPts = A.reg.nPts, nObs = A.obs.nObs, nTiles = A.pat.nTiles;
  const int32_t nT = A.lay.nT;
  for (int k = 0; k < 9; k++)
    if (upload(&d.var[k], h->data[k]) || alloc0(&d.varBak[k], h->data[k].size()) || upload(&d.redOf[k], A.lay.redOf[k]))
      return VB_E_HIP;
  if (upload(&d.rvKind, A.lay.rvKind) || upload(&d.rvHandle, A.lay.rvHandle) || upload(&d.rvDim, A.lay.rvDim) ||
      upload(&d.rvOff, A.lay.rvOff) || upload(&d.rvRowEnd, A.pat.rowEnd) || upload(&h->padRowsD, A.lay.padRows))
    return VB_E_HIP;
  {
    int8_t* co = nullptr;
    if (upload(&co, A.lay.colOwner)) return VB_E_HIP;
    d.colOwner = co;
  }
  if (upload(&d.obCostOrder, A.cost.order) || upload(&d.obPack, A.cost.pack) || upload(&d.obCP, A.cost.cp) ||
      upload(&d.obPose, A.obs.obPose) || upload(&d.obExtr, A.obs.obExtr) || upload(&d.obIntr, A.obs.obIntr) ||
      upload(&d.obVel, A.obs.obVel) || upload(&d.obRS, A.obs.obRS) || upload(&d.obPt, A.obs.obPt) ||
      upload(&d.obRed, A.obs.obRed) || upload(&d.obCol, A.pan.obCol) || upload(&d.obC, A.obs.obC) ||
      alloc0(&d.cache, nObs) || alloc0(&d.Jt, (size_t)kJPlanes * d.nObsPad))
    return VB_E_HIP;
  d.cacheW = d.cache;
  if (upload(&d.lmList, A.shard.lmList) || upload(&d.lmObs, A.obs.lmObs) || upload(&d.lmY, A.pan.lmY) ||
      upload(&d.lmBlk, A.pan.lmBlk) || upload(&d.blkRed, A.pan.blkRed) || upload(&d.blkCol, A.pan.blkCol) ||
      upload(&d.ptLm, A.reg.lmOfPoint) || upload(&d.pcRow, A.pan.pcRow) || upload(&d.pcBlk, A.pan.pcBlk) ||
      upload(&d.bxStart, A.pan.bxStart) || upload(&d.bxEnt, A.pan.bxEnt))
    return VB_E_HIP;
  if (alloc0(&d.Vchol, nPts * 6) || alloc0(&d.gp, nPts * 3) || alloc0(&d.z, nPts * 3) || alloc0(&d.xp, nPts * 3) ||
      alloc0(&d.Y, A.pan.lmY[nPts] + 128) || alloc0(&d.yZero, 256) ||
      alloc0(&d.gpNew, nPts * 3) || alloc0(&d.zNew, nPts * 3))
    return VB_E_HIP;
  if (upload(&d.oxStart, A.pan.oxStart) || upload(&d.oxObs, A.pan.oxObs) || upload(&d.oxSlot, A.pan.oxSlot) ||
      upload(&d.lxStart, A.pan.lxStart) || upload(&d.lxLm, A.pan.lxLm) || upload(&d.lxCol, A.pan.lxCol) ||
      upload(&d.lxChunk, A.pan.lxChunk))
    return VB_E_HIP;
  if (upload(&d.grpStart, A.schur.grpStart) || upload(&d.grpObs, A.schur.grpObs) || upload(&d.grpRed, A.schur.grpRed) ||
      upload(&d.schurRuns, A.schur.runs) || upload(&d.schurTasks, A.schur.tasks) || upload(&d.tileWorks, A.schur.works) ||
      upload(&d.tileEnts, A.schur.ents))
    return VB_E_HIP;
  if (A.schur.hasClear && upload(&h->clearTilesD, A.schur.clearTiles)) return VB_E_HIP;
  if (!h->shardTiles.empty() &&
      (upload(&h->shardTilesD, h->shardTiles) || alloc0(&h->shardPack, h->shardTiles.size() * (size_t)TS * TS)))
    return VB_E_HIP;
  if (upload(&d.tileIdx, A.pat.tileIdx) || alloc0(&d.tiles, (size_t)nTiles * TS * TS)) return VB_E_HIP;
  const size_t nPad = (size_t)nT * TS;
  if (alloc0(&d.gRed, nPad) || alloc0(&d.rhs, nPad) || alloc0(&d.xRed, nPad) || alloc0(&d.gRedNew, nPad) ||
      alloc0(&d.stepRed, nPad) || alloc0(&d.stepPt, nPts * 3) || alloc0(&d.subRed, nPad) ||
      alloc0(&d.subPt, nPts * 3) || alloc0(&h->yvec, nPad) || alloc0(&h->rhsWork, nPad))
    return VB_E_HIP;
  if (upload(&h->colStartD, h->colStart) || upload(&h->rowStartD, h->rowStart) || alloc0(&h->solveFlags, 4 * (size_t)nT) ||
      upload(&h->colTilesD, h->colTilesH) || upload(&h->colRowsD, h->colRowsH) || upload(&h->rowTilesD, h->rowTilesH) ||
      upload(&h->rowColD, h->rowColH) || alloc0(&h->dinv, (size_t)(nT + 1) * 1024) ||
      alloc0(&h->linv, (size_t)nT * TS * TS))
    return VB_E_HIP;
  for (int i = 0; i < 2; i++) {
    if (A.sch[i].built && uploadSched(A.sch[i], h->sch[i])) return VB_E_HIP;
    if (A.sn[i].built && uploadSnSched(A.sn[i], h->sn[i])) return VB_E_HIP;
    if (h->sch[i].nPtfDiag && !h->lscr && alloc0(&h->lscr, (size_t)nT * TS * TS)) return VB_E_HIP;
    if (h->sn[i].nCopy && !h->lscrSn && alloc0(&h->lscrSn, 2 * (size_t)nT * TS * TS)) return VB_E_HIP;
  }
  if (h->partSet) {
    if (upload(&h->ownRowsD, A.part.ownRows) || alloc0(&h->ownPack, A.part.ownRows.size() * (size_t)TS + 1) ||
        upload(&h->rootTilesD, h->rootTiles) || upload(&h->rootRowsD, h->rootRows) ||
        alloc0(&h->rootPack, h->rootTiles.size() * (size_t)TS * TS + 1) ||
        alloc0(&h->rowPack, h->rootRows.size() * (size_t)TS + 1))
      return VB_E_HIP;
  }
  for (int fk = 1; fk < 14; fk++)
    if (upload(&d.sf[fk].vars, h->fvars[fk]) || upload(&d.sf[fk].consts, A.small.consts[fk])) return VB_E_HIP;
  if ((h->isRoot || h->partSet) && d.nSmallStage > 0 &&
      (alloc0(&d.sJ, (size_t)d.nSmallStage * kSmallJ) || alloc0(&d.sE, (size_t)d.nSmallStage * kSmallE) ||
       alloc0(&d.sMeta, (size_t)d.nSmallStage * kSmallMeta)))
    return VB_E_HIP;
  if (A.preint.present) {
    h->pi.n = (int64_t)h->piSrc.size();
    if (upload(const_cast<PreintSrc**>(&h->pi.src), h->piSrc) || upload(const_cast<int64_t**>(&h->pi.t), A.preint.t) ||
        upload(const_cast<double**>(&h->pi.v), A.preint.v) || upload(const_cast<int64_t**>(&h->pi.off), A.preint.off) ||
        upload(const_cast<double**>(&h->pi.noise), A.preint.noise))
      return VB_E_HIP;
  }
  if (int rc = uploadRsTables(h)) return rc;
  if (alloc0(&d.red, 64) || alloc0(&d.redS, 2 * 64 * 8) || alloc0(&d.err, 8)) return VB_E_HIP;
  return 0;
}
}

int doFinalize(vb_handle h) {
  const Input in{h->data,    h->cst,     h->fvars,    h->fint,  h->fconst, h->cfg.imu_calib_options,
                 h->nRS,     h->sharded, h->lmBegin,  h->lmEnd, h->isRoot, h->partSet,
                 h->partRank, h->partWorld, h->piSrc, h->imuT,  h->imuV,   h->piT,
                 h->piV,     h->piNoise, readKnobs(*h)};
  Symbolic A;
  if (const Status e = analyze(in, A)) return fail(e.code, e.msg);
  copyToHandle(h, A);
  if (int rc = uploadAll(h, A)) return rc;
  h->finalized = true;
  return 0;
}

}
```

### visual_inertial_bundle_adjustment_amd/csrc/schur.hip

```cpp
#include "kernel_common.hpp"
#include <algorithm>

namespace viba {


__device__ __forceinline__ void landmark_eliminate(const Dev& d, double lambda, int mode, int64_t l) {
  const int lane = threadIdx.x & 63;
  const rec_t* Jt = d.Jt;
  const int64_t o0 = d.lmObs[l], o1 = d.lmObs[l + 1];
  double v00 = 0, v10 = 0, v20 = 0, v11 = 0, v21 = 0, v22 = 0, g0 = 0, g1 = 0, g2 = 0;
  for (int64_t o = o0 + lane; o < o1; o += 64) {
    const rec_t* r = Jt + o * kJA;
    const double e0 = r[kJe], e1 = r[kJe + 1];
    const double a0 = r[kJpt + 0], a1 = r[kJpt + 1], a2 = r[kJpt + 2];
    const double b0 = r[kJpt + 3], b1 = r[kJpt + 4], b2 = r[kJpt + 5];
    g0 += a0 * e0 + b0 * e1, g1 += a1 * e0 + b1 * e1, g2 += a2 * e0 + b2 * e1;
    if (mode == 0) {
      v00 += a0 * a0 + b0 * b0, v10 += a1 * a0 + b1 * b0, v20 += a2 * a0 + b2 * b0;
      v11 += a1 * a1 + b1 * b1, v21 += a2 * a1 + b2 * b1, v22 += a2 * a2 + b2 * b2;
    }
  }
  g0 = wave_sum(g0), g1 = wave_sum(g1), g2 = wave_sum(g2);
  if (mode == 1) {
    if (lane == 0) d.gpNew[l * 3] = g0, d.gpNew[l * 3 + 1] = g1, d.gpNew[l * 3 + 2] = g2;
    return;
  }
  v00 = wave_sum(v00), v10 = wave_sum(v10), v20 = wave_sum(v20);
  v11 = wave_sum(v11), v21 = wave_sum(v21), v22 = wave_sum(v22);
  v00 = v00 * (1.0 + lambda) + lambda;
  v11 = v11 * (1.0 + lambda) + lambda;
  v22 = v22 * (1.0 + lambda) + lambda;
  const double l00 = sqrt(v00);
  const double l10 = v10 / l00, l20 = v20 / l00;
  const double d11 = v11 - l10 * l10;
  const double l11 = sqrt(d11);
  const double l21 = (v21 - l20 * l10) / l11;
  const double d22 = v22 - l20 * l20 - l21 * l21;
  const double l22 = sqrt(d22);
  if (lane == 0) {
    if (!(v00 > 0) || !(d11 > 0) || !(d22 > 0)) atomicOr(d.err, 2);
    double* L = d.Vchol + l * 6;
    L[0] = l00, L[1] = l10, L[2] = l20, L[3] = l11, L[4] = l21, L[5] = l22;
    const double z0 = g0 / l00, z1 = (g1 - l10 * z0) / l11, z2 = (g2 - l20 * z0 - l21 * z1) / l22;
    d.z[l * 3] = z0, d.z[l * 3 + 1] = z1, d.z[l * 3 + 2] = z2;
    d.gp[l * 3] = g0, d.gp[l * 3 + 1] = g1, d.gp[l * 3 + 2] = g2;
  }
  const int64_t cb = d.lmY[l] / 3, ncol = d.lmY[l + 1] / 3 - cb;
  rec_t* Y = d.Y + d.lmY[l];
  for (int64_t c = lane; c < ncol; c += 64) {
    const int32_t b = d.pcBlk[cb + c];
    const int j = (int)(c - d.blkCol[b]);
    double w0 = 0, w1 = 0, w2 = 0;
    for (int64_t e = d.bxStart[b]; e < d.bxStart[b + 1]; e++) {
      const int32_t ent = d.bxEnt[e];
      const int s = ent & 3;
      const int64_t o = ent >> 2;
      const rec_t* r = Jt + o * kJA;
      const rec_t* x = jt_plane(Jt, d.nObsPad, o, slotPlane(s) + j);
      const double x0 = x[0], x1 = x[slotStride(s)];
      w0 += r[kJpt + 0] * x0 + r[kJpt + 3] * x1;
      w1 += r[kJpt + 1] * x0 + r[kJpt + 4] * x1;
      w2 += r[kJpt + 2] * x0 + r[kJpt + 5] * x1;
    }
    const double y0 = w0 / l00;
    const double y1 = (w1 - l10 * y0) / l11;
    const double y2 = (w2 - l20 * y0 - l21 * y1) / l22;
    Y[3 * c] = y0, Y[3 * c + 1] = y1, Y[3 * c + 2] = y2;
  }
}
__global__ void __launch_bounds__(256) landmark_kernel(Dev d, double lambda, int mode, int64_t lo, int64_t hi) {
  const int64_t l = lo + (int64_t)blockIdx.x * 4 + (threadIdx.x >> 6);
  if (l >= hi) return;
  landmark_eliminate(d, lambda, mode, l);
}

constexpr int kLmBigCols = 2048;

constexpr int kRecV = 16 / (int)sizeof(rec_t);
constexpr int kLmCh = VIBA_MIXED ? 6 : 4;
constexpr int kLmInA = (kLmCh * kJA / kRecV + 63) / 64;
constexpr int kLmInB = (kLmCh * kJB / kRecV + 63) / 64;
constexpr int kLmBOff = kLmInA * 64 * kRecV;
constexpr int kLmCOff = (kLmInA + kLmInB) * 64 * kRecV;
constexpr int kLmBuf = kLmCOff + 256 / (int)sizeof(rec_t);
static_assert(kLmCh * kJA <= kLmBOff, "region A of a chunk fits its DMA slots");

__device__ __forceinline__ void lm_issue(const Dev& d, int64_t oa, int nv, rec_t* buf, int lane) {
  const rec_t* gA = d.Jt + oa * kJA;
  const rec_t* gB = d.Jt + d.nObsPad * kJA + oa * kJB;
  const int vA = nv * (kJA / kRecV), vB = nv * (kJB / kRecV);
#pragma unroll
  for (int j = 0; j < kLmInA; j++) {
    const int p = j * 64 + lane;
    __builtin_amdgcn_global_load_lds((const __attribute__((address_space(1))) void*)(gA + (p < vA ? p : 0) * kRecV),
                                     (__attribute__((address_space(3))) void*)(buf + j * 64 * kRecV), 16, 0, 0);
  }
#pragma unroll
  for (int j = 0; j < kLmInB; j++) {
    const int p = j * 64 + lane;
    __builtin_amdgcn_global_load_lds((const __attribute__((address_space(1))) void*)(gB + (p < vB ? p : 0) * kRecV),
                                     (__attribute__((address_space(3))) void*)(buf + kLmBOff + j * 64 * kRecV), 16, 0, 0);
  }
  const int32_t* gC = d.obCol + oa * 4;
  __builtin_amdgcn_global_load_lds((const __attribute__((address_space(1))) void*)(gC + (lane < 4 * nv ? lane : 0)),
                                   (__attribute__((address_space(3))) void*)(buf + kLmCOff), 4, 0, 0);
}
__device__ __forceinline__ uint32_t lds_u32(const void* p) {
  return (uint32_t)(uintptr_t)(const __attribute__((address_space(3))) char*)p;
}
__device__ __forceinline__ void lm_read(const rec_t* ra, const rec_t* rx, const rec_t* rx1, const int32_t* rc,
                                        double (&a)[6], double& e0, double& e1, double& x0, double& x1, int32_t& pc) {
#if VIBA_MIXED
  float v[10];
  asm volatile(
      "ds_read_b32 %0, %11\n\tds_read_b32 %1, %11 offset:4\n\tds_read_b32 %2, %11 offset:8\n\t"
      "ds_read_b32 %3, %11 offset:12\n\tds_read_b32 %4, %11 offset:16\n\tds_read_b32 %5, %11 offset:20\n\t"
      "ds_read_b32 %6, %11 offset:24\n\tds_read_b32 %7, %11 offset:28\n\tds_read_b32 %8, %12\n\t"
      "ds_read_b32 %9, %13\n\tds_read_b32 %10, %14\n\ts_waitcnt lgkmcnt(0)"
      : "=&v"(v[0]), "=&v"(v[1]), "=&v"(v[2]), "=&v"(v[3]), "=&v"(v[4]), "=&v"(v[5]), "=&v"(v[6]), "=&v"(v[7]),
        "=&v"(v[8]), "=&v"(v[9]), "=&v"(pc)
      : "v"(lds_u32(ra)), "v"(lds_u32(rx)), "v"(lds_u32(rx1)), "v"(lds_u32(rc))
      : "memory");
#else
  double v[10];
  asm volatile(
      "ds_read_b64 %0, %11\n\tds_read_b64 %1, %11 offset:8\n\tds_read_b64 %2, %11 offset:16\n\t"
      "ds_read_b64 %3, %11 offset:24\n\tds_read_b64 %4, %11 offset:32\n\tds_read_b64 %5, %11 offset:40\n\t"
      "ds_read_b64 %6, %11 offset:48\n\tds_read_b64 %7, %11 offset:56\n\tds_read_b64 %8, %12\n\t"
      "ds_read_b64 %9, %13\n\tds_read_b32 %10, %14\n\ts_waitcnt lgkmcnt(0)"
      : "=&v"(v[0]), "=&v"(v[1]), "=&v"(v[2]), "=&v"(v[3]), "=&v"(v[4]), "=&v"(v[5]), "=&v"(v[6]), "=&v"(v[7]),
        "=&v"(v[8]), "=&v"(v[9]), "=&v"(pc)
      : "v"(lds_u32(ra)), "v"(lds_u32(rx)), "v"(lds_u32(rx1)), "v"(lds_u32(rc))
      : "memory");
#endif
  static_assert(kJe == 0 && kJpt == 2, "record planes 0..7: e, point Jacobian");
  e0 = v[0], e1 = v[1];
#pragma unroll
  for (int k = 0; k < 6; k++) a[k] = v[2 + k];
  x0 = v[8], x1 = v[9];
}

__device__ __forceinline__ void lm_stage_loop(const Dev& d, int64_t o0, int64_t n, rec_t* stg, double* W, int wave,
                                              int nwaves, int lane, double (&v)[9]) {
  const int nch = (int)((n + kLmCh - 1) / kLmCh);
  const int h = lane >> 5, jj = lane & 31;
  const int s = jj < 6 ? 0 : jj < 12 ? 1 : jj < 29 ? 2 : 3;
  const int j = jj - (s == 0 ? 0 : s == 1 ? 6 : s == 2 ? 12 : 29);
  const int pl = slotPlane(s) + j, st = slotStride(s);
  const int xo = pl < kJA ? pl : kLmBOff + (pl - kJA), xstep = pl < kJA ? kJA : kJB;
  auto nvOf = [&](int k) { return (int)min<int64_t>(n - (int64_t)k * kLmCh, kLmCh); };
  if (wave < nch) lm_issue(d, o0 + (int64_t)wave * kLmCh, nvOf(wave), stg, lane);
  for (int k = wave, b = 0; k < nch; k += nwaves, b ^= 1) {
    const int64_t ob = o0 + (int64_t)k * kLmCh;
    const int nv = nvOf(k);
    if (k + nwaves < nch) {
      lm_issue(d, ob + (int64_t)nwaves * kLmCh, nvOf(k + nwaves), stg + (b ^ 1) * kLmBuf, lane);
      asm volatile("s_waitcnt vmcnt(%0)" ::"n"(kLmInA + kLmInB + 1) : "memory");
    } else {
      asm volatile("s_waitcnt vmcnt(0)" ::: "memory");
    }
    const rec_t* S = stg + b * kLmBuf;
    for (int c = h; c < nv + (nv & 1); c += 2) {
      const int cc = min(c, nv - 1);
      double a[6], e0, e1, x0, x1;
      int32_t pc;
      lm_read(S + cc * kJA, S + xo + cc * xstep, S + xo + cc * xstep + st,
              reinterpret_cast<const int32_t*>(S + kLmCOff) + 4 * cc + s, a, e0, e1, x0, x1, pc);
      const bool valid = c < nv;
      if (valid && jj == 0) {
        v[6] += a[0] * e0 + a[3] * e1, v[7] += a[1] * e0 + a[4] * e1, v[8] += a[2] * e0 + a[5] * e1;
        v[0] += a[0] * a[0] + a[3] * a[3], v[1] += a[1] * a[0] + a[4] * a[3];
        v[2] += a[2] * a[0] + a[5] * a[3], v[3] += a[1] * a[1] + a[4] * a[4];
        v[4] += a[2] * a[1] + a[5] * a[4], v[5] += a[2] * a[2] + a[5] * a[5];
      }
      if (valid && pc >= 0 && j < (pc & 31)) {
        const int col = (pc >> 5) + j;
        const double w0 = a[0] * x0 + a[3] * x1, w1 = a[1] * x0 + a[4] * x1, w2 = a[2] * x0 + a[5] * x1;
        asm volatile("ds_add_f64 %0, %1\n\tds_add_f64 %0, %2 offset:8\n\tds_add_f64 %0, %3 offset:16"
                     ::"v"(lds_u32(W + 3 * col)), "v"(w0), "v"(w1), "v"(w2)
                     : "memory");
      }
    }
  }
  asm volatile("s_waitcnt vmcnt(0) lgkmcnt(0)" ::: "memory");
}

__global__ void __launch_bounds__(64) landmark_stage_kernel(Dev d, double lambda, int64_t first, int cap) {
  extern __shared__ __attribute__((aligned(16))) double lsm[];
  rec_t* stg = reinterpret_cast<rec_t*>(lsm);
  double* W = lsm + (2 * kLmBuf * (int)sizeof(rec_t) + 7) / 8;
  const int lane = threadIdx.x;
  const int64_t l = d.lmList[first + xcd_block(blockIdx.x, gridDim.x)];
  const int64_t o0 = d.lmObs[l], o1 = d.lmObs[l + 1], n = o1 - o0;
  const int64_t cb = d.lmY[l] / 3, ncol = d.lmY[l + 1] / 3 - cb;
  for (int i = lane; i < 3 * ncol; i += 64) W[i] = 0.0;
  asm volatile("s_waitcnt lgkmcnt(0)" ::: "memory");
  double v[9] = {0, 0, 0, 0, 0, 0, 0, 0, 0};
  lm_stage_loop(d, o0, n, stg, W, 0, 1, lane, v);
  double v00 = v[0], v10 = v[1], v20 = v[2], v11 = v[3], v21 = v[4], v22 = v[5], g0 = v[6], g1 = v[7], g2 = v[8];
  g0 = wave_sum(g0), g1 = wave_sum(g1), g2 = wave_sum(g2);
  v00 = wave_sum(v00), v10 = wave_sum(v10), v20 = wave_sum(v20);
  v11 = wave_sum(v11), v21 = wave_sum(v21), v22 = wave_sum(v22);
  v00 = v00 * (1.0 + lambda) + lambda;
  v11 = v11 * (1.0 + lambda) + lambda;
  v22 = v22 * (1.0 + lambda) + lambda;
  const double l00 = sqrt(v00);
  const double l10 = v10 / l00, l20 = v20 / l00;
  const double d11 = v11 - l10 * l10;
  const double l11 = sqrt(d11);
  const double l21 = (v21 - l20 * l10) / l11;
  const double d22 = v22 - l20 * l20 - l21 * l21;
  const double l22 = sqrt(d22);
  if (lane == 0) {
    if (!(v00 > 0) || !(d11 > 0) || !(d22 > 0)) atomicOr(d.err, 2);
    double* L = d.Vchol + l * 6;
    L[0] = l00, L[1] = l10, L[2] = l20, L[3] = l11, L[4] = l21, L[5] = l22;
    const double z0 = g0 / l00, z1 = (g1 - l10 * z0) / l11, z2 = (g2 - l20 * z0 - l21 * z1) / l22;
    d.z[l * 3] = z0, d.z[l * 3 + 1] = z1, d.z[l * 3 + 2] = z2;
    d.gp[l * 3] = g0, d.gp[l * 3 + 1] = g1, d.gp[l * 3 + 2] = g2;
  }
  __builtin_amdgcn_fence(__ATOMIC_RELEASE, "wavefront");
  __builtin_amdgcn_wave_barrier();
  __builtin_amdgcn_fence(__ATOMIC_ACQUIRE, "wavefront");
  rec_t* Y = d.Y + d.lmY[l];
  for (int64_t c = lane; c < ncol; c += 64) {
    const double y0 = W[3 * c] / l00;
    const double y1 = (W[3 * c + 1] - l10 * y0) / l11;
    const double y2 = (W[3 * c + 2] - l20 * y0 - l21 * y1) / l22;
    Y[3 * c] = y0, Y[3 * c + 1] = y1, Y[3 * c + 2] = y2;
  }
}

__global__ void __launch_bounds__(256) landmark_obs_wg_kernel(Dev d, double lambda, int64_t first, int cap) {
  extern __shared__ __attribute__((aligned(16))) double lsm[];
  __shared__ double part[4][9];
  __shared__ double Ls[6];
  const int tid = threadIdx.x, lane = tid & 63, wave = tid >> 6;
  rec_t* stg = reinterpret_cast<rec_t*>(lsm) + wave * 2 * kLmBuf;
  double* W = lsm + (8 * kLmBuf * (int)sizeof(rec_t) + 7) / 8;
  const int64_t l = d.lmList[first + blockIdx.x];
  const int64_t o0 = d.lmObs[l], o1 = d.lmObs[l + 1];
  const int64_t cb = d.lmY[l] / 3, ncol = d.lmY[l + 1] / 3 - cb;
  for (int i = tid; i < 3 * ncol; i += 256) W[i] = 0.0;
  __syncthreads();
  double v[9] = {0, 0, 0, 0, 0, 0, 0, 0, 0};
  lm_stage_loop(d, o0, o1 - o0, stg, W, wave, 4, lane, v);
#pragma unroll
  for (int k = 0; k < 9; k++) v[k] = wave_sum(v[k]);
  if (lane == 0)
#pragma unroll
    for (int k = 0; k < 9; k++) part[wave][k] = v[k];
  __syncthreads();
  if (tid == 0) {
#pragma unroll
    for (int k = 0; k < 9; k++) v[k] = part[0][k] + part[1][k] + part[2][k] + part[3][k];
    const double v00 = v[0] * (1.0 + lambda) + lambda, v11 = v[3] * (1.0 + lambda) + lambda;
    const double v22 = v[5] * (1.0 + lambda) + lambda;
    const double l00 = sqrt(v00);
    const double l10 = v[1] / l00, l20 = v[2] / l00;
    const double d11 = v11 - l10 * l10;
    const double l11 = sqrt(d11);
    const double l21 = (v[4] - l20 * l10) / l11;
    const double d22 = v22 - l20 * l20 - l21 * l21;
    const double l22 = sqrt(d22);
    if (!(v00 > 0) || !(d11 > 0) || !(d22 > 0)) atomicOr(d.err, 2);
    double* L = d.Vchol + l * 6;
    L[0] = Ls[0] = l00, L[1] = Ls[1] = l10, L[2] = Ls[2] = l20, L[3] = Ls[3] = l11, L[4] = Ls[4] = l21;
    L[5] = Ls[5] = l22;
    const double z0 = v[6] / l00, z1 = (v[7] - l10 * z0) / l11, z2 = (v[8] - l20 * z0 - l21 * z1) / l22;
    d.z[l * 3] = z0, d.z[l * 3 + 1] = z1, d.z[l * 3 + 2] = z2;
    d.gp[l * 3] = v[6], d.gp[l * 3 + 1] = v[7], d.gp[l * 3 + 2] = v[8];
  }
  __syncthreads();
  const double l00 = Ls[0], l10 = Ls[1], l20 = Ls[2], l11 = Ls[3], l21 = Ls[4], l22 = Ls[5];
  rec_t* Y = d.Y + d.lmY[l];
  for (int64_t c = tid; c < ncol; c += 256) {
    const double y0 = W[3 * c] / l00;
    const double y1 = (W[3 * c + 1] - l10 * y0) / l11;
    const double y2 = (W[3 * c + 2] - l20 * y0 - l21 * y1) / l22;
    Y[3 * c] = y0, Y[3 * c + 1] = y1, Y[3 * c + 2] = y2;
  }
}

__global__ void __launch_bounds__(256) landmark_list_kernel(Dev d, double lambda, int64_t first, int64_t n) {
  const int64_t li = (int64_t)blockIdx.x * 4 + (threadIdx.x >> 6);
  if (li >= n) return;
  landmark_eliminate(d, lambda, 0, d.lmList[first + li]);
}

__global__ void __launch_bounds__(256) landmark_z_kernel(Dev d, int64_t lo, int64_t hi) {
  const int64_t l = lo + (int64_t)blockIdx.x * blockDim.x + threadIdx.x;
  if (l >= hi) return;
  const double* L = d.Vchol + l * 6;
  const double* g = d.gpNew + l * 3;
  const double z0 = g[0] / L[0];
  const double z1 = (g[1] - L[1] * z0) / L[3];
  const double z2 = (g[2] - L[2] * z0 - L[4] * z1) / L[5];
  d.zNew[l * 3] = z0, d.zNew[l * 3 + 1] = z1, d.zNew[l * 3 + 2] = z2;
}



constexpr int kCh = kSchurCh;
constexpr int kTR = kSchurTR;

#ifndef VIBA_SCHUR_PF
#define VIBA_SCHUR_PF 0
#endif
#ifndef VIBA_SCHUR_WAVES
#define VIBA_SCHUR_WAVES (VIBA_SCHUR_PF ? 3 : 4)
#endif
__device__ __forceinline__ void load3(const double* p, double (&v)[3]) {
  typedef double d2u __attribute__((ext_vector_type(2), aligned(8)));
  const d2u x = *reinterpret_cast<const d2u*>(p);
  v[0] = x.x, v[1] = x.y, v[2] = p[2];
}
__device__ __forceinline__ void load3(const float* p, float (&v)[3]) {
  typedef float f3u __attribute__((ext_vector_type(3), aligned(4)));
  const f3u x = *reinterpret_cast<const f3u*>(p);
  v[0] = x.x, v[1] = x.y, v[2] = x.z;
// ... 77 lines not shown
#pragma unroll
    for (int i = 0; i < NR; i++)
#pragma unroll
      for (int b = 0; b < NBI; b++)
        if (!DIAG || a0 + i <= b) acc[i][b] = mfma_h(av[i], bv[b], acc[i][b]);
  };
  const int nl = rows / 3, nfull = (nl + 3) >> 2;
  constexpr bool PAIR = !DIAG && !VIBA_MIXED;
  auto ld3 = [&](int m, rec_t (&a3)[NR][3], rec_t (&b3)[NBI][3]) {
    const bool lv = 4 * m + l4 < nl;
    const uint2 c = lv ? ec[c0 + 4 * m + l4] : make_uint2(0u, 0u);
    const rec_t* base = lv ? Y : d.yZero;
    const rec_t* pJ = base + 3 * (int64_t)c.y;
    const rec_t* pI = base + 3 * (int64_t)c.x;
    if constexpr (PAIR && NR == 2) {
      load6(pJ + 3 * schur_row<NR, PAIR>(a0, 0, l15), a3[0], a3[1]);
    } else {
#pragma unroll
      for (int i = 0; i < NR; i++) load3(pJ + 3 * schur_row<NR, PAIR>(a0, i, l15), a3[i]);
    }
#pragma unroll
    for (int b = 0; b < NBI; b++) {
      if (PAIR && b < 2 * (NBI / 2)) {
        if ((b & 1) == 0) load6(pI + 3 * schur_col<NBI, PAIR>(b, l15), b3[b], b3[b + 1]);
      } else {
        load3(pI + 3 * schur_col<NBI, PAIR>(b, l15), b3[b]);
      }
    }
  };
  auto mm3 = [&](const rec_t (&a3)[NR][3], const rec_t (&b3)[NBI][3]) {
#pragma unroll
    for (int q = 0; q < 3; q++) {
      rec_t av[NR], bv[NBI];
#pragma unroll
      for (int i = 0; i < NR; i++) av[i] = a3[i][q];
#pragma unroll
      for (int b = 0; b < NBI; b++) bv[b] = b3[b][q];
      mm(av, bv);
    }
  };
#if VIBA_SCHUR_PF
  if (nfull > 0) {
    rec_t a3[NR][3], b3[NBI][3];
    ld3(0, a3, b3);
    for (int m = 0; m < nfull; m++) {
      rec_t a3n[NR][3], b3n[NBI][3];
      if (m + 1 < nfull) ld3(m + 1, a3n, b3n);
      mm3(a3, b3);
      if (m + 1 < nfull) {
#pragma unroll
        for (int i = 0; i < NR; i++)
#pragma unroll
          for (int q = 0; q < 3; q++) a3[i][q] = a3n[i][q];
#pragma unroll
        for (int b = 0; b < NBI; b++)
#pragma unroll
          for (int q = 0; q < 3; q++) b3[b][q] = b3n[b][q];
      }
    }
  }
#else
#pragma unroll 1
  for (int m = 0; m < nfull; m++) {
    rec_t a3[NR][3], b3[NBI][3];
    ld3(m, a3, b3);
    mm3(a3, b3);
    __builtin_amdgcn_sched_barrier(0);
  }
#endif
  schur_epilogue<NBI, NR, DIAG>(acc, a0, l4, l15, posI, posJ, nI, nJ, C);
}

__global__ void __launch_bounds__(256) __attribute__((amdgpu_waves_per_eu(VIBA_SCHUR_WAVES, VIBA_SCHUR_WAVES))) schur_run4_kernel(Dev d, double lambda) {
  __shared__ double C[TS * TS];
  __shared__ uint32_t ecol[256][2];
  __shared__ uint64_t rmask[256][2];
  __shared__ uint8_t posW[4][2][TS];
  __shared__ double rq[TS];
  const int64_t w = xcd_block(blockIdx.x, gridDim.x);
  const TileWork* wp = d.tileWorks + w;
  const TileWork wk = *wp;
  const bool diag = wk.I == wk.J;
  const int tid = threadIdx.x, lane = tid & 63, wave = __builtin_amdgcn_readfirstlane(tid >> 6);
  const int l15 = lane & 15, l4 = lane >> 4;
  const int cnt = wk.count;
  const TileEnt* ents = d.tileEnts + wk.start;
  if (tid < cnt) ecol[tid][0] = ents[tid].colI, ecol[tid][1] = ents[tid].colJ;
  if (tid < wk.nRuns) {
    const uint64_t* rm = d.schurRuns + 2 * ((int64_t)wk.runFirst + tid);
    rmask[tid][0] = rm[0], rmask[tid][1] = rm[1];
  }
  for (int i = tid; i < TS * TS; i += 256) C[i] = 0.0;
  if (tid < TS) rq[tid] = 0.0;
  __syncthreads();
  uint8_t* posI = posW[wave][0];
  uint8_t* posJ = posW[wave][1];
  const uint2* ec2 = reinterpret_cast<const uint2*>(&ecol[0][0]);
  const uint32_t* tasks = d.schurTasks + wk.taskFirst;
  const int tBeg = wp->wOff[wave], tEnd = wp->wOff[wave + 1];
  int cur = -1;
  for (int t = tBeg; t < tEnd; t++) {
    const uint32_t code = __builtin_amdgcn_readfirstlane(tasks[t]);
    const int r = code & 255, c0 = (code >> 8) & 255, nl = (code >> 16) & 63, a0 = (code >> 22) & 3;
    const uint64_t mI = uniform64(rmask[r][0]), mJ = uniform64(rmask[r][1]);
    const int nI = __popcll(mI), nJ = __popcll(mJ);
    const int nbI = (nI + 15) >> 4, nbJ = (nJ + 15) >> 4;
    if (r != cur) {
      __builtin_amdgcn_wave_barrier();
      if ((mI >> lane) & 1) posI[__popcll(mI & ((1ull << lane) - 1))] = (uint8_t)lane;
      if ((mJ >> lane) & 1) posJ[__popcll(mJ & ((1ull << lane) - 1))] = (uint8_t)lane;
      __builtin_amdgcn_fence(__ATOMIC_RELEASE, "wavefront");
      __builtin_amdgcn_wave_barrier();
      __builtin_amdgcn_fence(__ATOMIC_ACQUIRE, "wavefront");
      cur = r;
    }
    const int rows = 3 * nl;
    const int nr = min(kTR, nbJ - a0);
    const int sel = ((nbI - 1) * 2 + (nr - 1)) * 2 + (diag ? 1 : 0);
    switch (sel) {
#define VIBA_SCHUR_CASE(NBI, NR)                                                                      \
  case ((NBI - 1) * 2 + (NR - 1)) * 2:                                                                \
    schur_task<NBI, NR, false>(d, ec2, c0, rows, a0, l4, l15, posI, posJ, nI, nJ, C);                 \
    break;                                                                                            \
  case ((NBI - 1) * 2 + (NR - 1)) * 2 + 1:                                                            \
    schur_task<NBI, NR, true>(d, ec2, c0, rows, a0, l4, l15, posI, posJ, nI, nJ, C);                  \
    break;
      VIBA_SCHUR_CASE(1, 1) VIBA_SCHUR_CASE(2, 1) VIBA_SCHUR_CASE(3, 1) VIBA_SCHUR_CASE(4, 1)
#if VIBA_SCHUR_TR == 2
      VIBA_SCHUR_CASE(1, 2) VIBA_SCHUR_CASE(2, 2) VIBA_SCHUR_CASE(3, 2) VIBA_SCHUR_CASE(4, 2)
#endif
#undef VIBA_SCHUR_CASE
      default: break;
    }
    if (diag && a0 == 0 && lane < nI) schur_rhs(d, ecol, ents, c0, nl, lane, posI, rq);
  }
  __syncthreads();
  double* Ct = d.tiles + (int64_t)wk.tile * TS * TS;
  if (wk.kind == 1) {
    for (int i = tid; i < TS * TS; i += 256)
      if (C[i] != 0.0) atomicAdd(Ct + i, C[i]);
  } else if (wk.kind == 2) {
    for (int i = tid; i < TS * TS; i += 256) Ct[i] = C[i];
  } else {
    for (int i = tid; i < TS * TS; i += 256) Ct[i] += C[i];
  }
  if (diag && tid < TS) {
    const int64_t row = (int64_t)wk.I * TS + tid;
    if (row < d.nRed && rq[tid] != 0.0) atomicAdd(d.rhs + row, rq[tid]);
  }
}

constexpr int kGrpBase[4] = {0, 6, 12, 29};

__device__ __forceinline__ int grp_col_row(const Dev& d, const int32_t* red, int c, int& plane, int& stride) {
  const int s = c < 6 ? 0 : c < 12 ? 1 : c < 29 ? 2 : 3;
  const int j = c - kGrpBase[s];
  const int32_t X = red[s];
  plane = slotPlane(s) + j, stride = slotStride(s);
  if (X < 0 || j >= d.rvDim[X]) return -1;
  return (int)(d.rvOff[X] + j);
}

__device__ __forceinline__ void group_finish(const Dev& d, double lambda, int mode, int row0, int row1, const hacc4_t& a00,
                                             const hacc4_t& a10, const hacc4_t& a11, double g0, double g1, double* red) {
  const int tid = threadIdx.x, lane = tid & 63, wave = tid >> 6;
  const int l15 = lane & 15, l4 = lane >> 4;
  double* mine = red + (wave * 64 + lane) * 14;
#pragma unroll
  for (int k = 0; k < 4; k++) mine[k] = a00[k], mine[4 + k] = a10[k], mine[8 + k] = a11[k];
  mine[12] = g0, mine[13] = g1;
  __syncthreads();
  if (wave != 0) return;
  double t[14];
#pragma unroll
  for (int k = 0; k < 14; k++) t[k] = red[lane * 14 + k] + red[(64 + lane) * 14 + k] + red[(128 + lane) * 14 + k] + red[(192 + lane) * 14 + k];
  double gc0 = t[12], gc1 = t[13];
#pragma unroll
  for (int off = 16; off < 64; off += 16) {
    gc0 += __shfl(t[12], (lane + off) & 63, 64);
    gc1 += __shfl(t[13], (lane + off) & 63, 64);
  }
  double* gOut = mode == 0 ? d.gRed : d.gRedNew;
  if (l4 == 0) {
    if (row0 >= 0 && gc0 != 0.0) atomicAdd(gOut + row0, gc0);
    if (row1 >= 0 && gc1 != 0.0) atomicAdd(gOut + row1, gc1);
  }
  if (mode != 0) return;
  double* H = red;
#pragma unroll
  for (int k = 0; k < 4; k++) {
    const int m = kAccL4 * l4 + kAccR * k;
    H[m * 32 + l15] = t[k];
    H[(16 + m) * 32 + 16 + l15] = t[8 + k];
    H[(16 + m) * 32 + l15] = t[4 + k], H[l15 * 32 + 16 + m] = t[4 + k];
  }
  int32_t* ord = reinterpret_cast<int32_t*>(H + 32 * 32);
  int32_t* crow = ord + 32;
  int32_t* cu = crow + 32;
  int32_t* trow = cu + 32;
  int32_t* tpair = trow + 8;
  const int rowc = lane < 32 ? (lane < 16 ? row0 : row1) : -1;
  const bool val = rowc >= 0;
  int rank = 0;
  for (int c = 0; c < 32; c++) {
    const int rc = __builtin_amdgcn_readlane(rowc, c);
    if (rc >= 0 && rc < rowc) rank++;
  }
  const int nc = __popcll(__ballot(val));
  if (val) ord[rank] = lane;
  const int tr = rowc / TS;
  uint64_t left = __ballot(val);
  int nu = 0, u = -1;
  while (left) {
    const int tl = __builtin_amdgcn_readlane(tr, __builtin_ctzll(left));
    const bool hit = val && tr == tl;
    left &= ~__ballot(hit);
    if (hit) u = nu;
    if (lane == 0) trow[nu] = tl;
    nu++;
  }
  if (lane < 32) crow[lane] = rowc, cu[lane] = u;
  __builtin_amdgcn_wave_barrier();
  __builtin_amdgcn_fence(__ATOMIC_SEQ_CST, "workgroup");
  for (int q = lane; q < nu * nu; q += 64) {
    const int tu = trow[q / nu], tv = trow[q % nu];
    tpair[q] = tu >= tv ? d.tileIdx[(int64_t)tu * d.nT + tv] : -1;
  }
  __builtin_amdgcn_wave_barrier();
  __builtin_amdgcn_fence(__ATOMIC_SEQ_CST, "workgroup");
  const int P = nc * (nc + 1) / 2;
  for (int p = lane; p < P; p += 64) {
    const int q = P - 1 - p;
    int i = (int)((sqrtf(8.0f * q + 1.0f) - 1.0f) * 0.5f);
    while (i * (i + 1) / 2 > q) i--;
    while ((i + 1) * (i + 2) / 2 <= q) i++;
    const int b = nc - 1 - i, a = nc - 1 - (q - i * (i + 1) / 2);
    const int ca = ord[a], cb = ord[b];
    double v = H[ca * 32 + cb];
    if (v == 0.0) continue;
    const int R = crow[ca], C = crow[cb];
    if (a == b) v *= 1.0 + lambda;
    const int32_t ti = tpair[cu[ca] * nu + cu[cb]];
    if (ti >= 0) atomicAdd(d.tiles + (int64_t)ti * TS * TS + (C % TS) * TS + (R % TS), v);
    else atomicOr(d.err, 4);
  }
}

constexpr int kRecPieces = kJPlanes / kRecV;
constexpr int kGrpSkip = 8 / kRecV - 1;
constexpr int kGrpPieces = kRecPieces - kGrpSkip;
constexpr int kGrpPlanes = kGrpPieces * kRecV;
constexpr int kGrpShift = kGrpSkip * kRecV;
constexpr int kGrpLoads = VIBA_MIXED ? 3 : 4;
constexpr int kGrpChunk = kGrpLoads * 256 / kGrpPieces;
constexpr int kGrpStage = kGrpLoads * 256 * kRecV;
constexpr int kGrpIdx = 1024;
static_assert(kJA % kRecV == 0 && kJB % kRecV == 0, "record regions in whole 16 B pieces");
constexpr int kGrpLds = 2 * kGrpStage * (int)sizeof(rec_t) > 4 * 64 * 14 * 8 ? 2 * kGrpStage * (int)sizeof(rec_t) : 4 * 64 * 14 * 8;

__device__ __forceinline__ uint32_t lds_addr(const void* p) {
  return (uint32_t)(uintptr_t)(const __attribute__((address_space(3))) char*)p;
}
__device__ __forceinline__ void lds_read3(const double* a, const double* b, const double* c, double& x, double& y, double& z) {
  asm volatile("ds_read_b64 %0, %3\n\tds_read_b64 %1, %4\n\tds_read_b64 %2, %5\n\ts_waitcnt lgkmcnt(0)"
               : "=&v"(x), "=&v"(y), "=&v"(z)
               : "v"(lds_addr(a)), "v"(lds_addr(b)), "v"(lds_addr(c))
               : "memory");
}
__device__ __forceinline__ void lds_read3(const float* a, const float* b, const float* c, float& x, float& y, float& z) {
  asm volatile("ds_read_b32 %0, %3\n\tds_read_b32 %1, %4\n\tds_read_b32 %2, %5\n\ts_waitcnt lgkmcnt(0)"
               : "=&v"(x), "=&v"(y), "=&v"(z)
               : "v"(lds_addr(a)), "v"(lds_addr(b)), "v"(lds_addr(c))
               : "memory");
}

__device__ __forceinline__ void group_issue(const Dev& d, const int32_t* sIdx, int nv, rec_t* buf, int wave, int lane) {
#pragma unroll
  for (int j = 0; j < kGrpLoads; j++) {
    const int i = j * 256 + wave * 64 + lane;
    int c = i / kGrpPieces;
    const int qs = i - c * kGrpPieces;
    const int q = qs == 0 ? 0 : qs + kGrpSkip;
    if (c >= nv) c = 0;
    const int64_t o = sIdx[c];
    const rec_t* src = q < kJA / kRecV ? d.Jt + o * kJA + q * kRecV
                                        : d.Jt + d.nObsPad * kJA + o * kJB + (q - kJA / kRecV) * kRecV;
    __builtin_amdgcn_global_load_lds((const __attribute__((address_space(1))) void*)src,
                                     (__attribute__((address_space(3))) void*)(buf + (j * 256 + wave * 64) * kRecV), 16, 0, 0);
  }
}

__global__ void __launch_bounds__(256) obs_group_kernel(Dev d, double lambda, int mode) {
  __shared__ __attribute__((aligned(16))) double smem[kGrpLds / 8];
  __shared__ int32_t sIdx[kGrpIdx];
  rec_t* stg = reinterpret_cast<rec_t*>(smem);
  const int64_t g = xcd_block(blockIdx.x, gridDim.x);
  const int tid = threadIdx.x, lane = tid & 63, wave = __builtin_amdgcn_readfirstlane(tid >> 6);
  const int l15 = lane & 15, l4 = lane >> 4;
  const int32_t* rv = d.grpRed + 4 * g;
  int p0, s0, p1, s1;
  const int row0 = grp_col_row(d, rv, l15, p0, s0);
  const int row1 = grp_col_row(d, rv, 16 + l15, p1, s1);
  const int64_t o0 = d.grpStart[g], n = d.grpStart[g + 1] - o0;
  const int r = l4 & 1;
  const int q0 = row0 >= 0 ? p0 + r * s0 - kGrpShift : 0, q1 = row1 >= 0 ? p1 + r * s1 - kGrpShift : 0;
  hacc4_t a00 = {0, 0, 0, 0}, a10 = {0, 0, 0, 0}, a11 = {0, 0, 0, 0};
  double g0 = 0.0, g1 = 0.0;
  for (int64_t w0 = 0; w0 < n; w0 += kGrpIdx) {
    const int nw = (int)min<int64_t>(n - w0, kGrpIdx);
    for (int i = tid; i < nw; i += 256) sIdx[i] = d.grpObs[o0 + w0 + i];
    __syncthreads();
    const int nch = (nw + kGrpChunk - 1) / kGrpChunk;
    group_issue(d, sIdx, min(nw, kGrpChunk), stg, wave, lane);
    for (int k = 0; k < nch; k++) {
      const int c0 = k * kGrpChunk, nv = min(nw - c0, kGrpChunk);
      if (k + 1 < nch) {
        group_issue(d, sIdx + c0 + kGrpChunk, min(nw - c0 - kGrpChunk, kGrpChunk), stg + ((k + 1) & 1) * kGrpStage, wave, lane);
        asm volatile("s_waitcnt vmcnt(%0)" ::"n"(kGrpLoads) : "memory");
      } else {
        asm volatile("s_waitcnt vmcnt(0)" ::: "memory");
      }
      __builtin_amdgcn_s_barrier();
      __builtin_amdgcn_sched_barrier(0);
      const rec_t* S = stg + (k & 1) * kGrpStage;
      for (int ks = wave; 2 * ks < nv; ks += 4) {
        const int c = 2 * ks + (l4 >> 1);
        const rec_t* rc = S + min(c, nv - 1) * kGrpPlanes;
        rec_t er, v0, v1;
        lds_read3(rc + kJe + r, rc + q0, rc + q1, er, v0, v1);
        if (c >= nv) er = v0 = v1 = 0;
        if (row0 < 0) v0 = 0;
        if (row1 < 0) v1 = 0;
        g0 += (double)v0 * er, g1 += (double)v1 * er;
        if (mode == 0) {
          a00 = mfma_h(v0, v0, a00);
          a10 = mfma_h(v1, v0, a10);
          a11 = mfma_h(v1, v1, a11);
        }
      }
      __builtin_amdgcn_sched_barrier(0);
      __builtin_amdgcn_s_barrier();
    }
  }
  group_finish(d, lambda, mode, row0, row1, a00, a10, a11, g0, g1, smem);
}

__global__ void damp_small_kernel(Dev d, double lambda, int addIdentity) {
  const int64_t r = (int64_t)blockIdx.x * blockDim.x + threadIdx.x;
  if (r >= d.nRed || !owns_col(d, r / TS)) return;
  double* p = tile_ptr(d, r, r);
  *p = *p * (1.0 + lambda) + (addIdentity ? lambda : 0.0);
}

__global__ void __launch_bounds__(256) reduced_rhs_kernel(Dev d) {
  __shared__ double g[4][32];
  const int64_t* ch = d.lxChunk + 3 * (int64_t)blockIdx.x;
  const int X1 = (int)ch[0];
  const int d1 = d.rvDim[X1];
  const int64_t off1 = d.rvOff[X1];
  const int tid = threadIdx.x, lane = tid & 63, wave = tid >> 6;
  const int P = d1 <= 4 ? 4 : d1 <= 8 ? 8 : d1 <= 16 ? 16 : 32;
  const int S = 64 / P, slot = lane / P, j = lane % P;
  double acc = 0.0;
  for (int64_t idx = ch[1] + wave * S + slot; idx < ch[2]; idx += 4 * S) {
    const int64_t l = d.lxLm[idx];
    if (j >= d1 || l < d.lmB || l >= d.lmE) continue;
    const rec_t* y1 = d.Y + d.lmY[l] + 3 * (d.lxCol[idx] + j);
    acc += (double)y1[0] * d.zNew[l * 3] + (double)y1[1] * d.zNew[l * 3 + 1] + (double)y1[2] * d.zNew[l * 3 + 2];
  }
  for (int o = P; o < 64; o <<= 1) acc += __shfl_xor(acc, o, 64);
  if (lane < P && lane < d1) g[wave][lane] = acc;
  __syncthreads();
  if (tid < d1) atomicAdd(&d.rhs[off1 + tid], -(g[0][tid] + g[1][tid] + g[2][tid] + g[3][tid]));
}

void launch_axpby(double* y, const double* x, double a, double b, int64_t n, hipStream_t st);

void launch_landmark(const Dev& d, double lambda, int mode, int64_t lo, int64_t hi, hipStream_t st) {
  if (hi <= lo) return;
  if (mode == 2) {
    launchK(landmark_z_kernel, dim3(blocks(hi - lo, 256)), dim3(256), 0, st, d, lo, hi);
  } else if (mode == 0 && lo == d.lmB && hi == d.lmE) {
    if (d.nLmSmall)
      launchK(landmark_stage_kernel, dim3((unsigned)d.nLmSmall), dim3(64),
              (uint32_t)((2 * kLmBuf * sizeof(rec_t) + 7) / 8 * 8 + 3 * kLmSmallCols * sizeof(double)), st, d, lambda,
              (int64_t)0, kLmSmallCols);
    if (d.nLmBig && d.lmBigCols <= kLmBigCols)
      hipLaunchKernelGGL(landmark_obs_wg_kernel, dim3((unsigned)d.nLmBig), dim3(256),
                         (uint32_t)((8 * kLmBuf * sizeof(rec_t) + 7) / 8 * 8 + 3 * d.lmBigCols * sizeof(double)), st, d,
                         lambda, d.nLmSmall, (int)d.lmBigCols);
    else if (d.nLmBig)
      hipLaunchKernelGGL(landmark_list_kernel, dim3(blocks(d.nLmBig, 4)), dim3(256), 0, st, d, lambda, d.nLmSmall,
                         d.nLmBig);
  } else {
    launchK(landmark_kernel, dim3(blocks(hi - lo, 4)), dim3(256), 0, st, d, lambda, mode, lo, hi);
  }
}
void launch_damp(const Dev& d, double lambda, int addIdentity, hipStream_t st) {
  if (d.nRed) hipLaunchKernelGGL(damp_small_kernel, dim3(blocks(d.nRed, 256)), dim3(256), 0, st, d, lambda, addIdentity);
}
void launch_groups(const Dev& d, double lambda, hipStream_t st) {
  if (d.nGroups) hipLaunchKernelGGL(obs_group_kernel, dim3((unsigned)d.nGroups), dim3(256), 0, st, d, lambda, 0);
}
void launch_schur_products(const Dev& d, double lambda, hipStream_t st);
void launch_schur(const Dev& d, double lambda, int addIdentity, hipStream_t st) {
  launch_damp(d, lambda, addIdentity, st);
  launch_groups(d, lambda, st);
  launch_schur_products(d, lambda, st);
}
void launch_schur_products(const Dev& d, double lambda, hipStream_t st) {
  if (d.nTileWorks) launchK(schur_run4_kernel, dim3((unsigned)d.nTileWorks), dim3(256), 0, st, d, lambda);
  launch_axpby(d.rhs, d.gRed, 1.0, 1.0, d.nRed, st);
}
void launch_reduced_grad(const Dev& d, int mode, hipStream_t st) {
  if (mode == 0) {
    if (d.nGroups) hipLaunchKernelGGL(obs_group_kernel, dim3((unsigned)d.nGroups), dim3(256), 0, st, d, 0.0, 1);
    return;
  }
  (void)hipMemcpyAsync(d.rhs, d.gRedNew, (size_t)d.nT * TS * sizeof(double), hipMemcpyDeviceToDevice, st);
  if (d.nLxChunk) hipLaunchKernelGGL(reduced_rhs_kernel, dim3((unsigned)d.nLxChunk), dim3(256), 0, st, d);
}
}
```

Baseline: 57.42 LM iterations/s.

## Compress intrinsics Jacobian into generator terms and rebuild columns on the fly

Replaces the stored 34-entry intrinsics Jacobian with a compact set of generator values (weighted projection factors, theta powers, focal terms), shrinking the per-observation record from 72 to 64 planes. Consumers (Schur, landmark staging, observation-group kernels) reconstruct each intrinsics column on the fly from a few loads and a multiply-add, using a new per-observation camera code array. The aim is to cut memory traffic and footprint for the Jacobian store. In exchange the inner loops issue more LDS reads and do extra arithmetic per column, and several kernels now share more complex indexing.

```diff
diff --git a/visual_inertial_bundle_adjustment_amd/csrc/api.hip b/visual_inertial_bundle_adjustment_amd/csrc/api.hip
--- a/visual_inertial_bundle_adjustment_amd/csrc/api.hip
+++ b/visual_inertial_bundle_adjustment_amd/csrc/api.hip
@@ -546,7 +546,7 @@
   reportFree(h);
   Dev& d = h->d;
   void* ptrs[] = {d.rvKind, d.rvHandle, d.rvDim, d.rvOff, d.rvRowEnd, d.obCostOrder, d.obPack, d.obCP, d.obPose, d.obExtr, d.obIntr, d.obVel,
-                  d.obRS, d.obPt, d.obRed, d.obCol, d.obC, d.cache, d.Jt, d.lmObs, d.lmY, d.lmBlk, d.blkRed,
+                  d.obRS, d.obPt, d.obRed, d.obCol, d.obCam, d.obC, d.cache, d.Jt, d.lmObs, d.lmY, d.lmBlk, d.blkRed,
                   d.blkCol, d.pcRow, d.pcBlk, d.bxStart, d.bxEnt, d.Vchol, d.gp, d.z, d.xp, d.Y, d.yZero, d.gpNew, d.zNew, d.ptLm, d.oxStart, d.oxObs, d.oxSlot,
                   d.lxStart, d.lxLm, d.lxCol, d.lxChunk, d.tileWorks, d.schurRuns, d.schurTasks, d.tileEnts, d.grpStart, d.grpObs, d.grpRed, d.tileIdx, d.tiles, d.gRed, d.rhs, d.xRed, d.gRedNew, d.stepRed,
                   d.stepPt, d.subRed, d.subPt, d.lmList, d.rsOff, d.rsS, d.rsI, d.rsG, d.rsN, d.imuT, d.imuV, d.rsMid, d.rsHalf,
diff --git a/visual_inertial_bundle_adjustment_amd/csrc/device_math.hpp b/visual_inertial_bundle_adjustment_amd/csrc/device_math.hpp
--- a/visual_inertial_bundle_adjustment_amd/csrc/device_math.hpp
+++ b/visual_inertial_bundle_adjustment_amd/csrc/device_math.hpp
@@ -1,10 +1,12 @@
 #pragma once
 #include <hip/hip_runtime.h>
+#include "record.hpp"
 
 namespace viba {
 namespace dev {
 
 #define DEVI __device__ __forceinline__
+#define HDEVI __host__ __device__ __forceinline__
 
 struct q4 {
   double x, y, z, w;
@@ -223,7 +225,7 @@
 }
 
 template <bool WantJ>
-DEVI bool project(const double* cam, v3 pc, double uv[2], double Jc[6], double Jp[30]) {
+HDEVI bool project(const double* cam, v3 pc, double uv[2], double Jc[6], IntrGen& gen) {
   if (pc.z < 1e-6) return false;
   const double iz = 1.0 / pc.z;
   const double x = pc.x * iz, y = pc.y * iz;
@@ -235,10 +237,7 @@
     if (WantJ) {
       Jc[0] = p[0] * d00, Jc[1] = 0.0, Jc[2] = p[0] * d02;
       Jc[3] = 0.0, Jc[4] = p[1] * d11, Jc[5] = p[1] * d12;
-#pragma unroll
-      for (int i = 0; i < 30; i++) Jp[i] = 0.0;
-      Jp[0] = x, Jp[2] = 1;
-      Jp[16] = y, Jp[18] = 1;
+      gen = IntrGen{0.0, 0.0, 0.0, 0.0, x, y, 0.0, 0.0};
     }
     return true;
   }
@@ -247,10 +246,8 @@
   const double r2 = x * x + y * y, r = sqrt(r2);
   const double th = atan(r), th2 = th * th;
   double R = 1.0, dR = 0.0, t2i = th2;
-  double thp[6];
 #pragma unroll
   for (int i = 0; i < 6; i++) {
-    thp[i] = t2i;
     R += p[3 + i] * t2i;
     dR += p[3 + i] * 2.0 * (i + 1) * t2i;
     t2i *= th2;
@@ -283,19 +280,9 @@
     const double M10 = f * (D10 * G00 + D11 * G01), M11 = f * (D10 * G01 + D11 * G11);
     Jc[0] = M00 * d00, Jc[1] = M01 * d11, Jc[2] = M00 * d02 + M01 * d12;
     Jc[3] = M10 * d00, Jc[4] = M11 * d11, Jc[5] = M10 * d02 + M11 * d12;
-    Jp[0] = ud, Jp[15] = vd;
-    Jp[1] = 1, Jp[16] = 0, Jp[2] = 0, Jp[17] = 1;
     const double thdivr = (r < 1e-8) ? 1.0 : th / r;
-#pragma unroll
-    for (int i = 0; i < 6; i++) {
-      const double dxr = thdivr * thp[i] * x, dyr = thdivr * thp[i] * y;
-      Jp[3 + i] = f * (D00 * dxr + D01 * dyr);
-      Jp[18 + i] = f * (D10 * dxr + D11 * dyr);
-    }
-    Jp[9] = f * (2.0 * xr * xr + rr2), Jp[24] = f * (2.0 * xr * yr);
-    Jp[10] = f * (2.0 * xr * yr), Jp[25] = f * (2.0 * yr * yr + rr2);
-    Jp[11] = f * rr2, Jp[12] = f * rr4, Jp[13] = 0, Jp[14] = 0;
-    Jp[26] = 0, Jp[27] = 0, Jp[28] = f * rr2, Jp[29] = f * rr4;
+    const double dxr = thdivr * x, dyr = thdivr * y;
+    gen = IntrGen{ud, vd, f * (D00 * dxr + D01 * dyr), f * (D10 * dxr + D11 * dyr), xr, yr, th2, f};
   }
   return true;
 }
diff --git a/visual_inertial_bundle_adjustment_amd/csrc/engine.hpp b/visual_inertial_bundle_adjustment_amd/csrc/engine.hpp
--- a/visual_inertial_bundle_adjustment_amd/csrc/engine.hpp
+++ b/visual_inertial_bundle_adjustment_amd/csrc/engine.hpp
@@ -4,6 +4,7 @@
 #include <cstdint>
 #include <cstddef>
 #include <cstdlib>
+#include "record.hpp"
 
 namespace viba {
 
@@ -18,23 +19,6 @@
 
 constexpr int kLmSmallCols = 256;
 
-constexpr int kJe = 0;
-constexpr int kJpt = 2;
-constexpr int kJpose = 8;
-constexpr int kJextr = 20;
-constexpr int kJintr = 32;
-constexpr int kJvel = 66;
-constexpr int kJPlanes = 72;
-constexpr int kJA = 32, kJB = 40;
-template <typename T>
-__host__ __device__ inline T* jt_plane(T* Jt, int64_t nPad, int64_t o, int plane) {
-  return plane < kJA ? Jt + o * kJA + plane : Jt + nPad * kJA + o * kJB + (plane - kJA);
-}
-constexpr int kSlotPose = 0, kSlotExtr = 1, kSlotIntr = 2, kSlotVel = 3;
-__host__ __device__ inline int slotPlane(int s) {
-  return s == 0 ? kJpose : s == 1 ? kJextr : s == 2 ? kJintr : kJvel;
-}
-__host__ __device__ inline int slotStride(int s) { return s == 0 || s == 1 ? 6 : s == 2 ? 17 : 3; }
 
 struct ImuIdx {
   int gB, aB, gS, aS, gN, aN, rT, gaT, size;
@@ -105,6 +89,7 @@
   int32_t* obPack = nullptr;
   double* obCP = nullptr;
   int32_t* obCol = nullptr;
+  int32_t* obCam = nullptr;
   double* obC = nullptr;
   double* cache = nullptr;
   double* cacheW = nullptr;
diff --git a/visual_inertial_bundle_adjustment_amd/csrc/factors.hip b/visual_inertial_bundle_adjustment_amd/csrc/factors.hip
--- a/visual_inertial_bundle_adjustment_amd/csrc/factors.hip
+++ b/visual_inertial_bundle_adjustment_amd/csrc/factors.hip
@@ -36,7 +36,7 @@
 struct VisOut {
   double e[2];
   double Jpt[6], Jpose[12], Jextr[12], Jvel[6];
-  double* Jintr;
+  double* G;
 };
 
 template <bool WantJ, bool PointOnly = false>
@@ -44,8 +44,9 @@
                          VisOut& o) {
   v3 pRig = se3_act(Tbw, X);
   v3 pCam = se3_act(Tcb, pRig);
-  double uv[2], Jc[6], Jp[30];
-  if (!project<WantJ>(cam, pCam, uv, Jc, Jp)) return false;
+  double uv[2], Jc[6];
+  IntrGen gen;
+  if (!project<WantJ>(cam, pCam, uv, Jc, gen)) return false;
   const double s00 = obsC[2], s01 = obsC[3], s10 = obsC[4], s11 = obsC[5];
   const double r0 = uv[0] - obsC[0], r1 = uv[1] - obsC[1];
   o.e[0] = s00 * r0 + s01 * r1;
@@ -79,14 +80,10 @@
       o.Jextr[r * 6 + 5] = B[0] * mc.y - B[1] * mc.x;
     }
     if (PointOnly) return true;
-    const int n = (int)cam[1];
-#pragma unroll
-    for (int j = 0; j < 17; j++) {
-      const bool in = j < 15 && j < n;
-      const double a0 = in ? Jp[j < 15 ? j : 0] : 0.0, a1 = in ? Jp[15 + (j < 15 ? j : 0)] : 0.0;
-      o.Jintr[j] = s00 * a0 + s01 * a1;
-      o.Jintr[17 + j] = s10 * a0 + s11 * a1;
-    }
+    o.G[0] = gen.ud, o.G[1] = gen.vd, o.G[2] = gen.qx, o.G[3] = gen.qy;
+    o.G[4] = gen.xr, o.G[5] = gen.yr, o.G[6] = gen.th2, o.G[7] = gen.f;
+#pragma unroll
+    for (int i = 0; i < 4; i++) o.G[8 + i] = 0.0;
   }
   return true;
 }
@@ -112,7 +109,6 @@
     double Jt[12];
 #pragma unroll
     for (int i = 0; i < 12; i++) Jt[i] = o.Jpose[i];
-    const int n = (int)cam[1];
     const bool estRO = cam[7] != 0.0, estOff = cam[8] != 0.0;
     if (wantTime && (estRO || estOff)) {
       const double kEps = 1e-6;
@@ -129,11 +125,11 @@
         for (int k = 0; k < 6; k++) s += Jt[r * 6 + k] * (lg[k] / kEps);
         dE[r] = s;
       }
-      const int iRO = estRO ? n : -1, iOff = estOff ? n + (estRO ? 1 : 0) : -1;
-#pragma unroll
-      for (int j = 0; j < 17; j++) {
-        if (j == iOff) o.Jintr[j] = -dE[0], o.Jintr[17 + j] = -dE[1];
-        if (j == iRO) o.Jintr[j] = dE[0] * tpf, o.Jintr[17 + j] = dE[1] * tpf;
+      const int iRO = estRO ? 0 : -1, iOff = estOff ? (estRO ? 1 : 0) : -1;
+#pragma unroll
+      for (int j = 0; j < 2; j++) {
+        if (j == iOff) o.G[8 + 2 * j] = -dE[0], o.G[9 + 2 * j] = -dE[1];
+        if (j == iRO) o.G[8 + 2 * j] = dE[0] * tpf, o.G[9 + 2 * j] = dE[1] * tpf;
       }
     }
     double M[36];
@@ -177,7 +173,7 @@
 template <bool Cost>
 __global__ void __launch_bounds__(kVisBlock) visual_lin_kernel(Dev d, int updateCache, int dontRetry, int64_t lo,
                                                                int64_t hi) {
-  __shared__ double stage[kVisBlock / 64][64 * kJB];
+  __shared__ double stage[kVisBlock / 64][64 * (kJA + 1)];
   const int lane = threadIdx.x & 63, wave = threadIdx.x >> 6;
   const int64_t ob = lo + (int64_t)blockIdx.x * kVisBlock + wave * 64;
   const int nrec = (int)max<int64_t>(0, min<int64_t>(64, hi - ob));
@@ -188,7 +184,7 @@
   double acc[1] = {0.0};
   double cst[4] = {0.0, 0.0, 0.0, 0.0};
   VisOut v;
-  v.Jintr = S + lane * kJB;
+  v.G = S + lane * (kJB + 1);
   bool ok = false;
   double w = 0.0;
   if (lane < nrec) {
@@ -235,11 +231,20 @@
     }
   }
   if (lane < nrec) {
-    double* r = S + lane * kJB;
-#pragma unroll
-    for (int i = 0; i < 34; i++) r[i] = ok ? w * r[i] : 0.0;
-#pragma unroll
-    for (int i = 0; i < 6; i++) r[kJvel - kJA + i] = ok ? w * v.Jvel[i] : 0.0;
+    double* r = S + lane * (kJB + 1);
+    if (ok) {
+      const double* obsC = d.obCP + (ob + lane) * 6;
+      const IntrGen gen{r[0], r[1], r[2], r[3], r[4], r[5], r[6], r[7]};
+      double rs[4], vel[6];
+#pragma unroll
+      for (int i = 0; i < 4; i++) rs[i] = w * r[8 + i];
+#pragma unroll
+      for (int i = 0; i < 6; i++) vel[i] = w * v.Jvel[i];
+      pack_region_b(r, gen, d.var[4][(int64_t)pb.x * 24] != 0.0, w * obsC[2], w * obsC[3], w * obsC[4], w * obsC[5], rs, vel);
+    } else {
+#pragma unroll
+      for (int i = 0; i < kJB; i++) r[i] = 0.0;
+    }
   }
   __builtin_amdgcn_fence(__ATOMIC_RELEASE, "wavefront");
   __builtin_amdgcn_wave_barrier();
@@ -250,7 +255,7 @@
     for (int q0 = 0; q0 < nq; q0 += 64) {
       const int q = q0 + lane, r = min(q / (kJB / 2), 63), c = 2 * (q % (kJB / 2));
       const int64_t orec = __shfl(o, r, 64);
-      if (q < nq) store_planes(dst + orec * kJB + c, S[r * kJB + c], S[r * kJB + c + 1]);
+      if (q < nq) store_planes(dst + orec * kJB + c, S[r * (kJB + 1) + c], S[r * (kJB + 1) + c + 1]);
     }
   }
   __builtin_amdgcn_fence(__ATOMIC_RELEASE, "wavefront");
@@ -300,7 +305,7 @@
     const int4 pa = reinterpret_cast<const int4*>(d.obPack)[2 * i], pb = reinterpret_cast<const int4*>(d.obPack)[2 * i + 1];
     const int64_t o = pa.x;
     VisOut v;
-    v.Jintr = nullptr;
+    v.G = nullptr;
     bool oor = false, ok;
     const double* obsC = d.obCP + i * 6;
     const double* Xp = d.var[0] + (int64_t)pa.y * 3;
@@ -342,7 +347,7 @@
     const int64_t i = Hist ? t : posOfRow[R.first + t];
     const int4 pa = reinterpret_cast<const int4*>(d.obPack)[2 * i], pb = reinterpret_cast<const int4*>(d.obPack)[2 * i + 1];
     VisOut v;
-    v.Jintr = nullptr;
+    v.G = nullptr;
     v.e[0] = v.e[1] = 0.0;
     bool oor = false, ok;
     const double* obsC = d.obCP + i * 6;
@@ -1072,7 +1077,7 @@
   double c = 0, g0 = 0, g1 = 0, g2 = 0, h00 = 0, h10 = 0, h20 = 0, h11 = 0, h21 = 0, h22 = 0;
   for (int64_t q = lane; q < n; q += 64) {
     VisOut v;
-    v.Jintr = nullptr;
+    v.G = nullptr;
     if (!refine_eval<true>(d, obs[q], X, v)) {
       if (update) bk[q] = -1.0;
       continue;
@@ -1100,7 +1105,7 @@
   for (int64_t q = lane; q < n; q += 64) {
     if (bk[q] < 0) continue;
     VisOut v;
-    v.Jintr = nullptr;
+    v.G = nullptr;
     if (!refine_eval<false>(d, obs[q], X, v)) {
       c += bk[q];
       continue;
diff --git a/visual_inertial_bundle_adjustment_amd/csrc/finalize.hip b/visual_inertial_bundle_adjustment_amd/csrc/finalize.hip
--- a/visual_inertial_bundle_adjustment_amd/csrc/finalize.hip
+++ b/visual_inertial_bundle_adjustment_amd/csrc/finalize.hip
@@ -135,6 +135,11 @@
       alloc0(&d.cache, nObs) || alloc0(&d.Jt, (size_t)kJPlanes * d.nObsPad))
     return VB_E_HIP;
   d.cacheW = d.cache;
+  {
+    std::vector<int32_t> obCam((size_t)nObs);
+    for (int64_t o = 0; o < nObs; o++) obCam[o] = viba::cam_code(&h->data[4][(size_t)A.obs.obIntr[o] * 24]);
+    if (upload(&d.obCam, obCam)) return VB_E_HIP;
+  }
   if (upload(&d.lmList, A.shard.lmList) || upload(&d.lmObs, A.obs.lmObs) || upload(&d.lmY, A.pan.lmY) ||
       upload(&d.lmBlk, A.pan.lmBlk) || upload(&d.blkRed, A.pan.blkRed) || upload(&d.blkCol, A.pan.blkCol) ||
       upload(&d.ptLm, A.reg.lmOfPoint) || upload(&d.pcRow, A.pan.pcRow) || upload(&d.pcBlk, A.pan.pcBlk) ||
diff --git a/visual_inertial_bundle_adjustment_amd/csrc/record.hpp b/visual_inertial_bundle_adjustment_amd/csrc/record.hpp
--- /dev/null
+++ b/visual_inertial_bundle_adjustment_amd/csrc/record.hpp
@@ -0,0 +1,102 @@
+#pragma once
+#include <cstdint>
+
+#if defined(__HIPCC__)
+#define VIBA_HD __host__ __device__ inline
+#else
+#define VIBA_HD inline
+#endif
+
+namespace viba {
+
+constexpr int kJe = 0;
+constexpr int kJpt = 2;
+constexpr int kJpose = 8;
+constexpr int kJextr = 20;
+constexpr int kJintr = 32;
+constexpr int kJvel = 56;
+constexpr int kJPlanes = 64;
+constexpr int kJA = 32, kJB = 32;
+constexpr int kGV = 0, kGth = 10, kGf2 = 16, kGf4 = 17, kGbx = 18, kGby = 19, kGrs = 20;
+constexpr int kGvel = kJvel - kJA;
+static_assert(kJA + kJB == kJPlanes && kJintr == kJA && kGrs + 4 == kGvel && kGvel + 6 + 2 == kJB, "record layout");
+static_assert(kJA % 4 == 0 && kJB % 4 == 0, "both regions in whole 16 B pieces, double and float");
+
+template <typename T>
+VIBA_HD T* jt_plane(T* Jt, int64_t nPad, int64_t o, int plane) {
+  return plane < kJA ? Jt + o * kJA + plane : Jt + nPad * kJA + o * kJB + (plane - kJA);
+}
+constexpr int kSlotPose = 0, kSlotExtr = 1, kSlotIntr = 2, kSlotVel = 3;
+VIBA_HD int slotPlane(int s) { return s == 0 ? kJpose : s == 1 ? kJextr : s == 2 ? kJintr : kJvel; }
+VIBA_HD int slotStride(int s) { return s == 0 || s == 1 ? 6 : s == 2 ? 1 : 3; }
+
+VIBA_HD int cam_code(const double* cam) { return (int)cam[1]; }
+
+struct ColOp {
+  int pa, pb, ka, kb, step;
+  bool one, hasb;
+};
+VIBA_HD ColOp col_op(int s, int j) {
+  ColOp c;
+  if (s != kSlotIntr) {
+    c.pa = c.pb = c.ka = c.kb = slotPlane(s) + j, c.step = slotStride(s), c.one = true, c.hasb = false;
+    return c;
+  }
+  const int v = j == 0 ? 2 : j <= 2 ? j - 1 : j <= 8 ? 3 : (j == 9 || j == 11 || j == 12) ? 0 : 1;
+  c.pa = kJintr + kGV + 2 * v, c.pb = kJintr + kGV + 2 * 4, c.step = 1;
+  c.ka = kJintr + (j <= 8 ? kGth + (j >= 3 ? j - 3 : 0) : (j == 12 || j == 14) ? kGf4 : kGf2);
+  c.kb = kJintr + (j == 10 ? kGby : kGbx);
+  c.one = j <= 2, c.hasb = j == 9 || j == 10;
+  return c;
+}
+VIBA_HD double col_value(const ColOp& c, bool intr, int j, int n, double va, double vb, double ka, double kb, double rs0,
+                         double rs1) {
+  const double gen = (c.one ? va : ka * va) + (c.hasb ? kb * vb : 0.0);
+  const bool live = j < n && j < 15;
+  return !intr ? va : live ? gen : j == n ? rs0 : j == n + 1 ? rs1 : 0.0;
+}
+
+struct IntrGen {
+  double ud, vd, qx, qy, xr, yr, th2, f;
+};
+
+VIBA_HD void pack_region_b(double* B, const IntrGen& g, bool fish, double a00, double a01, double a10, double a11,
+                           const double rs[4], const double vel[6]) {
+  double* V = B + kGV;
+  if (fish) {
+    V[0] = a00, V[1] = a10, V[2] = a01, V[3] = a11;
+    V[4] = a00 * g.ud + a01 * g.vd, V[5] = a10 * g.ud + a11 * g.vd;
+    V[6] = a00 * g.qx + a01 * g.qy, V[7] = a10 * g.qx + a11 * g.qy;
+    V[8] = a00 * g.xr + a01 * g.yr, V[9] = a10 * g.xr + a11 * g.yr;
+    double p = g.th2;
+#pragma unroll
+    for (int i = 0; i < 6; i++) B[kGth + i] = p, p *= g.th2;
+    const double rr2 = g.xr * g.xr + g.yr * g.yr, rr4 = rr2 * rr2;
+    B[kGf2] = g.f * rr2, B[kGf4] = g.f * rr4, B[kGbx] = 2.0 * g.f * g.xr, B[kGby] = 2.0 * g.f * g.yr;
+  } else {
+    V[4] = a00 * g.xr, V[5] = a10 * g.xr;
+    V[0] = a01 * g.yr, V[1] = a11 * g.yr;
+    V[2] = a00, V[3] = a10;
+    V[6] = a01, V[7] = a11;
+    V[8] = V[9] = 0.0;
+    B[kGth] = 1.0;
+#pragma unroll
+    for (int i = 1; i < 10; i++) B[kGth + i] = 0.0;
+  }
+#pragma unroll
+  for (int i = 0; i < 4; i++) B[kGrs + i] = rs[i];
+#pragma unroll
+  for (int i = 0; i < 6; i++) B[kGvel + i] = vel[i];
+  B[kGvel + 6] = B[kGvel + 7] = 0.0;
+}
+
+template <typename T>
+VIBA_HD void intr_column(const T* B, int n, int j, double& c0, double& c1) {
+  const ColOp c = col_op(kSlotIntr, j);
+  const T *va = B + (c.pa - kJA), *vb = B + (c.pb - kJA);
+  const double ka = (double)B[c.ka - kJA], kb = (double)B[c.kb - kJA];
+  c0 = col_value(c, true, j, n, (double)va[0], (double)vb[0], ka, kb, (double)B[kGrs], (double)B[kGrs + 2]);
+  c1 = col_value(c, true, j, n, (double)va[1], (double)vb[1], ka, kb, (double)B[kGrs + 1], (double)B[kGrs + 3]);
+}
+
+}
diff --git a/visual_inertial_bundle_adjustment_amd/csrc/schur.hip b/visual_inertial_bundle_adjustment_amd/csrc/schur.hip
--- a/visual_inertial_bundle_adjustment_amd/csrc/schur.hip
+++ b/visual_inertial_bundle_adjustment_amd/csrc/schur.hip
@@ -56,8 +56,13 @@
       const int s = ent & 3;
       const int64_t o = ent >> 2;
       const rec_t* r = Jt + o * kJA;
-      const rec_t* x = jt_plane(Jt, d.nObsPad, o, slotPlane(s) + j);
-      const double x0 = x[0], x1 = x[slotStride(s)];
+      double x0, x1;
+      if (s == kSlotIntr) {
+        intr_column(Jt + d.nObsPad * kJA + o * kJB, d.obCam[o], j, x0, x1);
+      } else {
+        const rec_t* x = jt_plane(Jt, d.nObsPad, o, slotPlane(s) + j);
+        x0 = x[0], x1 = x[slotStride(s)];
+      }
       w0 += r[kJpt + 0] * x0 + r[kJpt + 3] * x1;
       w1 += r[kJpt + 1] * x0 + r[kJpt + 4] * x1;
       w2 += r[kJpt + 2] * x0 + r[kJpt + 5] * x1;
@@ -82,6 +87,7 @@
 constexpr int kLmInB = (kLmCh * kJB / kRecV + 63) / 64;
 constexpr int kLmBOff = kLmInA * 64 * kRecV;
 constexpr int kLmCOff = (kLmInA + kLmInB) * 64 * kRecV;
+static_assert(5 * kLmCh <= 64, "the chunk's index words in one load");
 constexpr int kLmBuf = kLmCOff + 256 / (int)sizeof(rec_t);
 static_assert(kLmCh * kJA <= kLmBOff, "region A of a chunk fits its DMA slots");
 
@@ -101,43 +107,46 @@
     __builtin_amdgcn_global_load_lds((const __attribute__((address_space(1))) void*)(gB + (p < vB ? p : 0) * kRecV),
                                      (__attribute__((address_space(3))) void*)(buf + kLmBOff + j * 64 * kRecV), 16, 0, 0);
   }
-  const int32_t* gC = d.obCol + oa * 4;
-  __builtin_amdgcn_global_load_lds((const __attribute__((address_space(1))) void*)(gC + (lane < 4 * nv ? lane : 0)),
+  const int lc = lane - 4 * kLmCh;
+  const int32_t* gC = lc < 0 ? d.obCol + oa * 4 + (lane < 4 * nv ? lane : 0) : d.obCam + oa + (lc < nv ? lc : 0);
+  __builtin_amdgcn_global_load_lds((const __attribute__((address_space(1))) void*)gC,
                                    (__attribute__((address_space(3))) void*)(buf + kLmCOff), 4, 0, 0);
 }
 __device__ __forceinline__ uint32_t lds_u32(const void* p) {
   return (uint32_t)(uintptr_t)(const __attribute__((address_space(3))) char*)p;
 }
-__device__ __forceinline__ void lm_read(const rec_t* ra, const rec_t* rx, const rec_t* rx1, const int32_t* rc,
-                                        double (&a)[6], double& e0, double& e1, double& x0, double& x1, int32_t& pc) {
 #if VIBA_MIXED
-  float v[10];
-  asm volatile(
-      "ds_read_b32 %0, %11\n\tds_read_b32 %1, %11 offset:4\n\tds_read_b32 %2, %11 offset:8\n\t"
-      "ds_read_b32 %3, %11 offset:12\n\tds_read_b32 %4, %11 offset:16\n\tds_read_b32 %5, %11 offset:20\n\t"
-      "ds_read_b32 %6, %11 offset:24\n\tds_read_b32 %7, %11 offset:28\n\tds_read_b32 %8, %12\n\t"
-      "ds_read_b32 %9, %13\n\tds_read_b32 %10, %14\n\ts_waitcnt lgkmcnt(0)"
-      : "=&v"(v[0]), "=&v"(v[1]), "=&v"(v[2]), "=&v"(v[3]), "=&v"(v[4]), "=&v"(v[5]), "=&v"(v[6]), "=&v"(v[7]),
-        "=&v"(v[8]), "=&v"(v[9]), "=&v"(pc)
-      : "v"(lds_u32(ra)), "v"(lds_u32(rx)), "v"(lds_u32(rx1)), "v"(lds_u32(rc))
-      : "memory");
+#define VIBA_LM_RD "ds_read_b32 "
+#define VIBA_LM_OFF(k) " offset:" #k "*4\n\t"
 #else
-  double v[10];
-  asm volatile(
-      "ds_read_b64 %0, %11\n\tds_read_b64 %1, %11 offset:8\n\tds_read_b64 %2, %11 offset:16\n\t"
-      "ds_read_b64 %3, %11 offset:24\n\tds_read_b64 %4, %11 offset:32\n\tds_read_b64 %5, %11 offset:40\n\t"
-      "ds_read_b64 %6, %11 offset:48\n\tds_read_b64 %7, %11 offset:56\n\tds_read_b64 %8, %12\n\t"
-      "ds_read_b64 %9, %13\n\tds_read_b32 %10, %14\n\ts_waitcnt lgkmcnt(0)"
-      : "=&v"(v[0]), "=&v"(v[1]), "=&v"(v[2]), "=&v"(v[3]), "=&v"(v[4]), "=&v"(v[5]), "=&v"(v[6]), "=&v"(v[7]),
-        "=&v"(v[8]), "=&v"(v[9]), "=&v"(pc)
-      : "v"(lds_u32(ra)), "v"(lds_u32(rx)), "v"(lds_u32(rx1)), "v"(lds_u32(rc))
-      : "memory");
+#define VIBA_LM_RD "ds_read_b64 "
+#define VIBA_LM_OFF(k) " offset:" #k "*8\n\t"
 #endif
+__device__ __forceinline__ void lm_read(const rec_t* ra, const rec_t* ra0, const rec_t* ra1, const rec_t* rb, const rec_t* rka,
+                                        const rec_t* rkb, const rec_t* rrs, const int32_t* rc, const int32_t* rn,
+                                        double (&a)[6], double& e0, double& e1, double (&x)[4], double& ka, double& kb,
+                                        double (&rs)[4], int32_t& pc, int32_t& n) {
+  rec_t v[18];
+  asm volatile(VIBA_LM_RD "%0, %20" VIBA_LM_OFF(0) VIBA_LM_RD "%1, %20" VIBA_LM_OFF(1) VIBA_LM_RD "%2, %20" VIBA_LM_OFF(2)
+               VIBA_LM_RD "%3, %20" VIBA_LM_OFF(3) VIBA_LM_RD "%4, %20" VIBA_LM_OFF(4) VIBA_LM_RD "%5, %20" VIBA_LM_OFF(5)
+               VIBA_LM_RD "%6, %20" VIBA_LM_OFF(6) VIBA_LM_RD "%7, %20" VIBA_LM_OFF(7)
+               VIBA_LM_RD "%8, %21\n\t" VIBA_LM_RD "%9, %22\n\t" VIBA_LM_RD "%10, %23" VIBA_LM_OFF(0) VIBA_LM_RD "%11, %23" VIBA_LM_OFF(1)
+               VIBA_LM_RD "%12, %24\n\t" VIBA_LM_RD "%13, %25\n\t"
+               VIBA_LM_RD "%14, %26" VIBA_LM_OFF(0) VIBA_LM_RD "%15, %26" VIBA_LM_OFF(1) VIBA_LM_RD "%16, %26" VIBA_LM_OFF(2)
+               VIBA_LM_RD "%17, %26" VIBA_LM_OFF(3) "ds_read_b32 %18, %27\n\tds_read_b32 %19, %28\n\ts_waitcnt lgkmcnt(0)"
+               : "=&v"(v[0]), "=&v"(v[1]), "=&v"(v[2]), "=&v"(v[3]), "=&v"(v[4]), "=&v"(v[5]), "=&v"(v[6]), "=&v"(v[7]),
+                 "=&v"(v[8]), "=&v"(v[9]), "=&v"(v[10]), "=&v"(v[11]), "=&v"(v[12]), "=&v"(v[13]), "=&v"(v[14]), "=&v"(v[15]),
+                 "=&v"(v[16]), "=&v"(v[17]), "=&v"(pc), "=&v"(n)
+               : "v"(lds_u32(ra)), "v"(lds_u32(ra0)), "v"(lds_u32(ra1)), "v"(lds_u32(rb)), "v"(lds_u32(rka)), "v"(lds_u32(rkb)),
+                 "v"(lds_u32(rrs)), "v"(lds_u32(rc)), "v"(lds_u32(rn))
+               : "memory");
   static_assert(kJe == 0 && kJpt == 2, "record planes 0..7: e, point Jacobian");
   e0 = v[0], e1 = v[1];
 #pragma unroll
   for (int k = 0; k < 6; k++) a[k] = v[2 + k];
-  x0 = v[8], x1 = v[9];
+#pragma unroll
+  for (int k = 0; k < 4; k++) x[k] = v[8 + k], rs[k] = v[14 + k];
+  ka = v[12], kb = v[13];
 }
 
 __device__ __forceinline__ void lm_stage_loop(const Dev& d, int64_t o0, int64_t n, rec_t* stg, double* W, int wave,
@@ -146,8 +155,10 @@
   const int h = lane >> 5, jj = lane & 31;
   const int s = jj < 6 ? 0 : jj < 12 ? 1 : jj < 29 ? 2 : 3;
   const int j = jj - (s == 0 ? 0 : s == 1 ? 6 : s == 2 ? 12 : 29);
-  const int pl = slotPlane(s) + j, st = slotStride(s);
-  const int xo = pl < kJA ? pl : kLmBOff + (pl - kJA), xstep = pl < kJA ? kJA : kJB;
+  const ColOp op = col_op(s, j);
+  auto staged = [](int p) { return p < kJA ? p : kLmBOff + (p - kJA); };
+  const int xstep = op.pa < kJA ? kJA : kJB;
+  const int xa = staged(op.pa), xb = staged(op.pb), xka = staged(op.ka), xkb = staged(op.kb), xrs = staged(kJintr + kGrs);
   auto nvOf = [&](int k) { return (int)min<int64_t>(n - (int64_t)k * kLmCh, kLmCh); };
   if (wave < nch) lm_issue(d, o0 + (int64_t)wave * kLmCh, nvOf(wave), stg, lane);
   for (int k = wave, b = 0; k < nch; k += nwaves, b ^= 1) {
@@ -160,12 +171,15 @@
       asm volatile("s_waitcnt vmcnt(0)" ::: "memory");
     }
     const rec_t* S = stg + b * kLmBuf;
+    const int32_t* SC = reinterpret_cast<const int32_t*>(S + kLmCOff);
     for (int c = h; c < nv + (nv & 1); c += 2) {
       const int cc = min(c, nv - 1);
-      double a[6], e0, e1, x0, x1;
-      int32_t pc;
-      lm_read(S + cc * kJA, S + xo + cc * xstep, S + xo + cc * xstep + st,
-              reinterpret_cast<const int32_t*>(S + kLmCOff) + 4 * cc + s, a, e0, e1, x0, x1, pc);
+      double a[6], e0, e1, xv[4], ka, kb, rs[4];
+      int32_t pc, nl;
+      lm_read(S + cc * kJA, S + xa + cc * xstep, S + xa + cc * xstep + op.step, S + xb + cc * xstep, S + xka + cc * xstep,
+              S + xkb + cc * xstep, S + xrs + cc * kJB, SC + 4 * cc + s, SC + 4 * kLmCh + cc, a, e0, e1, xv, ka, kb, rs, pc, nl);
+      const double x0 = col_value(op, s == kSlotIntr, j, nl, xv[0], xv[2], ka, kb, rs[0], rs[2]);
+      const double x1 = col_value(op, s == kSlotIntr, j, nl, xv[1], xv[3], ka, kb, rs[1], rs[3]);
       const bool valid = c < nv;
       if (valid && jj == 0) {
         v[6] += a[0] * e0 + a[3] * e1, v[7] += a[1] * e0 + a[4] * e1, v[8] += a[2] * e0 + a[5] * e1;
@@ -549,11 +563,15 @@
 
 constexpr int kGrpBase[4] = {0, 6, 12, 29};
 
-__device__ __forceinline__ int grp_col_row(const Dev& d, const int32_t* red, int c, int& plane, int& stride) {
+__device__ __forceinline__ int grp_col_row(const Dev& d, const int32_t* red, int c, int n, ColOp& op) {
   const int s = c < 6 ? 0 : c < 12 ? 1 : c < 29 ? 2 : 3;
   const int j = c - kGrpBase[s];
   const int32_t X = red[s];
-  plane = slotPlane(s) + j, stride = slotStride(s);
+  op = col_op(s, j);
+  if (s == kSlotIntr && !(j < n && j < 15)) {
+    op.pa = op.pb = op.ka = op.kb = kJintr + kGrs + 2 * min(max(j - n, 0), 1);
+    op.one = true, op.hasb = false;
+  }
   if (X < 0 || j >= d.rvDim[X]) return -1;
   return (int)(d.rvOff[X] + j);
 }
@@ -658,16 +676,20 @@
 __device__ __forceinline__ uint32_t lds_addr(const void* p) {
   return (uint32_t)(uintptr_t)(const __attribute__((address_space(3))) char*)p;
 }
-__device__ __forceinline__ void lds_read3(const double* a, const double* b, const double* c, double& x, double& y, double& z) {
-  asm volatile("ds_read_b64 %0, %3\n\tds_read_b64 %1, %4\n\tds_read_b64 %2, %5\n\ts_waitcnt lgkmcnt(0)"
-               : "=&v"(x), "=&v"(y), "=&v"(z)
-               : "v"(lds_addr(a)), "v"(lds_addr(b)), "v"(lds_addr(c))
-               : "memory");
-}
-__device__ __forceinline__ void lds_read3(const float* a, const float* b, const float* c, float& x, float& y, float& z) {
-  asm volatile("ds_read_b32 %0, %3\n\tds_read_b32 %1, %4\n\tds_read_b32 %2, %5\n\ts_waitcnt lgkmcnt(0)"
-               : "=&v"(x), "=&v"(y), "=&v"(z)
-               : "v"(lds_addr(a)), "v"(lds_addr(b)), "v"(lds_addr(c))
+#if VIBA_MIXED
+#define VIBA_GRP_RD "ds_read_b32 "
+#else
+#define VIBA_GRP_RD "ds_read_b64 "
+#endif
+__device__ __forceinline__ void lds_read9(const rec_t* e, const rec_t* a0, const rec_t* b0, const rec_t* ka0, const rec_t* kb0,
+                                          const rec_t* a1, const rec_t* b1, const rec_t* ka1, const rec_t* kb1, rec_t& er,
+                                          rec_t (&x)[8]) {
+  asm volatile(VIBA_GRP_RD "%0, %9\n\t" VIBA_GRP_RD "%1, %10\n\t" VIBA_GRP_RD "%2, %11\n\t" VIBA_GRP_RD "%3, %12\n\t"
+               VIBA_GRP_RD "%4, %13\n\t" VIBA_GRP_RD "%5, %14\n\t" VIBA_GRP_RD "%6, %15\n\t" VIBA_GRP_RD "%7, %16\n\t"
+               VIBA_GRP_RD "%8, %17\n\ts_waitcnt lgkmcnt(0)"
+               : "=&v"(er), "=&v"(x[0]), "=&v"(x[1]), "=&v"(x[2]), "=&v"(x[3]), "=&v"(x[4]), "=&v"(x[5]), "=&v"(x[6]), "=&v"(x[7])
+               : "v"(lds_addr(e)), "v"(lds_addr(a0)), "v"(lds_addr(b0)), "v"(lds_addr(ka0)), "v"(lds_addr(kb0)), "v"(lds_addr(a1)),
+                 "v"(lds_addr(b1)), "v"(lds_addr(ka1)), "v"(lds_addr(kb1))
                : "memory");
 }
 
@@ -695,12 +717,14 @@
   const int tid = threadIdx.x, lane = tid & 63, wave = __builtin_amdgcn_readfirstlane(tid >> 6);
   const int l15 = lane & 15, l4 = lane >> 4;
   const int32_t* rv = d.grpRed + 4 * g;
-  int p0, s0, p1, s1;
-  const int row0 = grp_col_row(d, rv, l15, p0, s0);
-  const int row1 = grp_col_row(d, rv, 16 + l15, p1, s1);
+  const int code = rv[kSlotIntr] >= 0 ? cam_code(d.var[4] + (int64_t)d.rvHandle[rv[kSlotIntr]] * 24) : 0;
+  ColOp op0, op1;
+  const int row0 = grp_col_row(d, rv, l15, code, op0);
+  const int row1 = grp_col_row(d, rv, 16 + l15, code, op1);
   const int64_t o0 = d.grpStart[g], n = d.grpStart[g + 1] - o0;
   const int r = l4 & 1;
-  const int q0 = row0 >= 0 ? p0 + r * s0 - kGrpShift : 0, q1 = row1 >= 0 ? p1 + r * s1 - kGrpShift : 0;
+  const int qa0 = op0.pa + r * op0.step - kGrpShift, qb0 = op0.pb + r - kGrpShift, qk0 = op0.ka - kGrpShift, ql0 = op0.kb - kGrpShift;
+  const int qa1 = op1.pa + r * op1.step - kGrpShift, qb1 = op1.pb + r - kGrpShift, qk1 = op1.ka - kGrpShift, ql1 = op1.kb - kGrpShift;
   hacc4_t a00 = {0, 0, 0, 0}, a10 = {0, 0, 0, 0}, a11 = {0, 0, 0, 0};
   double g0 = 0.0, g1 = 0.0;
   for (int64_t w0 = 0; w0 < n; w0 += kGrpIdx) {
@@ -723,8 +747,10 @@
       for (int ks = wave; 2 * ks < nv; ks += 4) {
         const int c = 2 * ks + (l4 >> 1);
         const rec_t* rc = S + min(c, nv - 1) * kGrpPlanes;
-        rec_t er, v0, v1;
-        lds_read3(rc + kJe + r, rc + q0, rc + q1, er, v0, v1);
+        rec_t er, x[8];
+        lds_read9(rc + kJe + r, rc + qa0, rc + qb0, rc + qk0, rc + ql0, rc + qa1, rc + qb1, rc + qk1, rc + ql1, er, x);
+        rec_t v0 = (op0.one ? x[0] : x[2] * x[0]) + (op0.hasb ? x[3] * x[1] : (rec_t)0);
+        rec_t v1 = (op1.one ? x[4] : x[6] * x[4]) + (op1.hasb ? x[7] * x[5] : (rec_t)0);
         if (c >= nv) er = v0 = v1 = 0;
         if (row0 < 0) v0 = 0;
         if (row1 < 0) v1 = 0;
```

After: 57.88 LM iterations/s, median of 6. Within noise of the previous version (+0.8%).
